# pkusys/Auncel

Hardware: AMD Instinct MI355X
Metric: queries/sec @ recall@10>=0.95, SIFT-10M d=128 IVF4096, 1/2/4/8 GPU (higher is better)
Workload: dtype u8

## Files before the change

### auncel_amd/csrc/ivf_engine.hip

```cpp
#include <hip/hip_runtime.h>

#include <algorithm>
#include <atomic>
#include <cfloat>
#include <cmath>
#include <cstdlib>
#include <chrono>
#include <condition_variable>
#include <deque>
#include <functional>
#include <map>
#include <cstring>
#include <memory>
#include <stdexcept>
#include <string>
#include <mutex>
#include <thread>
#include <unordered_set>
#include <vector>

#include "../../include/auncel_amd.h"
#include "exact_args.h"
#include "ivf_kernels.h"
#include "kmeans_host.h"
// ... 1760 lines not shown
            ra.stage = h->c_stage.as<uint32_t>();
            ra.nscan = h->c_nscan.as<unsigned long long>();
            ra.done = h->c_done.as<uint32_t>();
            ra.D = d_out_dis + c0 * nprobe;
            ra.I = d_out_keys + c0 * nprobe;
            ra.stats = h->w_misc.as<unsigned long long>();
            ra.error = reinterpret_cast<uint32_t*>(h->w_misc.as<unsigned long long>() + STATS_ROWS * 4);
            launch_replay(ra, s);
        } else {
            bool tail_neutral = false;
            if (sort_rows_ranks_a_prefix((uint32_t)nlist, (uint32_t)nprobe, (uint32_t)prefix) && c0 == 0 && m == n && d_out_dis == h->w_cdis.p &&
                d_out_keys == h->w_ckeys.p) {
                amd_ivf::CoarseTail& ct = h->coarse_tail;
                tail_neutral = ct.valid && ct.dis == d_out_dis && ct.keys == d_out_keys && ct.prefix == prefix && ct.nprobe == nprobe && ct.rows >= n &&
                               ct.metric == h->metric && ct.touch_dis + 1 == h->w_cdis.touch && ct.touch_keys + 1 == h->w_ckeys.touch &&
                               !getenv("AUNCEL_AMD_WRITE_TAILS");
                ct = amd_ivf::CoarseTail{true, d_out_dis, d_out_keys, prefix, nprobe, tail_neutral ? ct.rows : n, h->metric, h->w_cdis.touch, h->w_ckeys.touch};
            } else {
                h->coarse_tail.valid = false;
            }
            launch_sort_rows(h->w_dist.as<float>(), (uint32_t)m, (uint32_t)nlist, (uint32_t)nprobe, h->metric,
                             d_out_dis + c0 * nprobe, d_out_keys + c0 * nprobe, s, (uint32_t)prefix, tail_neutral);
            if (heap_ties) {
                if (!h->w_tie_rows.p) {
                    h->w_tie_rows.ensure(8);
                    HIP_CHECK(hipMemsetAsync(h->w_tie_rows.p, 0, 8, s));
                }
                const size_t nout = prefix && prefix < nprobe ? prefix : nprobe;
                const bool ran = launch_heap_tie_order(h->w_dist.as<float>(), (uint32_t)m, (uint32_t)nlist, (uint32_t)nprobe, (uint32_t)nout,
                                                       h->metric, d_out_dis + c0 * nprobe, d_out_keys + c0 * nprobe,
                                                       h->w_tie_rows.as<unsigned long long>(), s);
                if (!ran && (h->ties_override == 1 || ties_opt == 1))
                    throw EngineError("coarse tie order by the reference's heap needs nlist x 12 bytes of LDS (nlist <= ~13 000)");
            }
        }
        h->timer.end(t, s);
        if (!cached || c0 + m < n) {
            HIP_CHECK(stream_sync(s));
            if (c0 == 0 && m == n) {
                h->coarse_sig = csig;
                h->coarse_sig_valid = true;
            }
        }
    }
}

TunerDev make_tuner(amd_ivf* h, size_t query_topk, float multipler, float std_m, const float* d_req, const float* d_gt,
                    unsigned long long* d_np, float* d_tr, int profile) {
    TunerDev t{};
    t.enabled = 1;
    t.profile = profile & 1;
    t.overhead = (profile & 2) ? 1 : 0;
    t.max_topk = (uint32_t)ix(h)->tuner_max_topk;
    t.query_topk = (uint32_t)query_topk;
    t.ntraces = (uint32_t)ix(h)->tuner_ntraces;
    t.multipler = multipler;
    t.std_m = std_m;
    t.interdis = ix(h)->d_interdis.as<float>();
    t.arcos = ix(h)->d_arcos.as<float>();
    t.trace_off = ix(h)->d_trace_off.as<uint32_t>();
    t.trace_x = ix(h)->d_trace_x.as<float>();
    t.trace_y = ix(h)->d_trace_y.as<float>();
    t.trace_std = ix(h)->d_trace_std.as<float>();
    t.require_acc = d_req;
    t.gt_D = d_gt;
    t.my_nprobe = d_np;
    t.t_recalls = d_tr;
    return t;
}

void run_rounds_device(amd_ivf* h, const RoundSpec& base, size_t n, size_t first_round_in, size_t total_nprobe,
                       const unsigned long long* d_np_abs ) {
    amd_ivf* I = ix(h);
    size_t first_round = first_round_in;
    const size_t nlist = h->nlist;
    hipStream_t s = h->stream;
    static const bool sync_env = getenv("AUNCEL_AMD_SYNC_ROUNDS") != nullptr || getenv("AUNCEL_AMD_DEBUG_REPLAY") != nullptr;
    const bool chained = !(base.range || base.d_budget_ms || sync_env);
    const double grow_env = opt(h, OPT_ROUND_GROW, 0.0);
    const bool filter_ok = filter_available(h, I, base.bytes) && !base.range;
    const bool filter_half = filter_ok && ensure_frag16(I);
    if (filter_ok && !filter_half) ensure_frag32(I);
    const float* lanes = base.bytes ? nullptr : ensure_lanes(I);
    struct Fp32Gate {
        amd_ivf* ix;
        bool held;
        Fp32Gate(amd_ivf* index, bool wanted) : ix(index), held(false) {
            if (!wanted || (int)index->opt.get(OPT_FP32_IN_FLIGHT, 4) <= 0) return;
            std::unique_lock<std::mutex> lk(ix->fp32_gate_mu);
            const uint64_t mine = ix->fp32_gate_next++;
            ix->fp32_gate_cv.wait(lk, [&] {
                const int limit = (int)ix->opt.get(OPT_FP32_IN_FLIGHT, 4);
                return mine == ix->fp32_gate_serving && (limit <= 0 || ix->fp32_running < limit);
            });
            ix->fp32_gate_serving++;
            ix->fp32_running++;
            held = true;
            lk.unlock();
            ix->fp32_gate_cv.notify_all();
        }
        ~Fp32Gate() {
            if (!held) return;
            {
                std::lock_guard<std::mutex> lk(ix->fp32_gate_mu);
                ix->fp32_running--;
            }
            ix->fp32_gate_cv.notify_all();
        }
    } fp32_gate(I, !base.bytes && n >= 256);
    if (filter_ok && base.tuner.enabled) first_round = filter_first_probes(I, (size_t)base.k, 64, 0.015);
    const double grow = grow_env > 0 ? grow_env : base.bytes ? 12.0 : filter_ok ? 6.0 : 3.5;
    size_t seg_cap = (size_t)2 << 20;
    if (!base.bytes) {
        const size_t groups = ((size_t)4 << 30) / ((size_t)h->dpad * SCAN_RQ * sizeof(float));
        seg_cap = std::min(seg_cap, std::max<size_t>((size_t)64 << 10, (groups > nlist ? groups - nlist : 0) * SCAN_RQ));
    }
    size_t maxlist = 0;
    for (size_t l = 0; l < nlist; l++) maxlist = std::max<size_t>(maxlist, I->h_list_off[l + 1] - I->h_list_off[l]);
    const size_t item_cap = (seg_cap / 32 + nlist) * ((maxlist + SCAN_WAVE_VECS - 1) / SCAN_WAVE_VECS) + nlist * 4 + 16;
    static const size_t seg_cap_env = getenv("AUNCEL_AMD_SEG_CAP_PAIRS") ? (size_t)atol(getenv("AUNCEL_AMD_SEG_CAP_PAIRS")) : 0;
    const size_t round_pairs = seg_cap_env ? std::min(seg_cap, std::max(seg_cap_env, total_nprobe)) : seg_cap;
    static const size_t budget_env = getenv("AUNCEL_AMD_DIST_BUDGET_MB") ? (size_t)atol(getenv("AUNCEL_AMD_DIST_BUDGET_MB")) << 18 : 0;
    const size_t padded_max = (maxlist + 1023) & ~(size_t)1023;
    const double all_rows = (double)n * (double)std::min<size_t>(total_nprobe, nlist) * (double)padded_max;
    size_t budget = budget_env ? budget_env : std::max<size_t>(h->dist_budget_floats, (size_t)2 << 30);
    const uint64_t bsig = (uint64_t)n * 1000003u ^ (uint64_t)first_round_in * 10007u ^ (uint64_t)total_nprobe * 101u ^ (base.bytes ? 1u : 0u) ^
                          (base.tuner.enabled ? 2u : 0u) ^ (base.train.enabled ? 4u : 0u) ^ ((uint64_t)base.k << 40);
    if (!budget_env && chained && base.tuner.enabled) {
        size_t want;
        size_t known = h->dist_want.get(bsig);
        {
            amd_ivf* owner = ix(h);
            std::lock_guard<std::mutex> lock(owner->want_mu);
            known = std::max(known, owner->shared_want.get(bsig));
        }
        if (known) {
            want = known + known / 4;
        } else {
            const double first = (double)n * (double)std::min<size_t>(std::max<size_t>(first_round_in, 1), std::min<size_t>(total_nprobe, nlist)) * (double)padded_max;
            want = (size_t)std::min<double>(first * (1.0 + 0.25 * grow), (double)budget);
        }
        budget = std::min(budget, std::max<size_t>(want, (size_t)16 << 20));
    }
    if (all_rows < (double)budget) budget = (size_t)all_rows + 64;
    budget = std::max<size_t>(budget, I->h_list_off[nlist] + 1024 * nlist + 1024);
    if (filter_ok && budget > ((size_t)1 << 31)) budget = (size_t)1 << 31;
    if (base.bytes && budget > ((size_t)1 << 31)) throw std::runtime_error("distance rows beyond 2^31 floats (byte-code scan offsets are 32-bit)");
    static const bool no_thr = getenv("AUNCEL_AMD_NO_THRESHOLD") != nullptr;
    h->w_pl_pad.ensure(n * 4);
    h->w_mask.ensure((budget / 64 + 2 + 256) * 8);
    const int row_lists_opt = (int)opt(h, OPT_ROW_LISTS, ROW_LISTS_DEFAULT);
    static const size_t row_lists_min = getenv("AUNCEL_AMD_ROW_LISTS_MIN") ? (size_t)atoi(getenv("AUNCEL_AMD_ROW_LISTS_MIN")) : 256;
    const bool row_lists = row_lists_opt != 0 && n >= row_lists_min;
    if (row_lists) {
        h->w_cl_cnt.ensure(seg_cap * 4);
        h->w_cl_ent.ensure((seg_cap + 64) * CL_CAP * sizeof(uint2));
        h->w_cl_arena.ensure((size_t)CL_ARENA * sizeof(uint2));
        h->w_cl_cursor.ensure(8 * 32 * 4);
    }
    h->w_pl_cnt.ensure(n * 4);
    h->w_pl_need.ensure(n * 8);
    h->w_seg_begin.ensure(n * 4);
    h->w_pl_dist_base.ensure(n * 8);
    h->w_qsel.ensure(n * 4);
    h->w_seg_list.ensure(seg_cap * 4);
    h->w_seg_off.ensure(seg_cap * 8);
    h->w_pair_query.ensure(seg_cap * 4);
    h->w_pair_out.ensure(seg_cap * 8);
    h->w_group_p0.ensure(seg_cap * 4);
    h->w_group_cnt.ensure(seg_cap * 4);
    h->w_items.ensure(item_cap * sizeof(ScanItem));
    h->w_pl_lcount.ensure(nlist * 4);
    h->w_pl_lstart.ensure(nlist * 4);
    h->w_pl_gbase.ensure(nlist * 4);
    h->w_pl_ibase.ensure(4 * nlist * 4);
    h->w_pl_fill.ensure(8 * nlist * 4);
    h->w_seg_slot.ensure(seg_cap * 4);
    constexpr size_t CNT_WORDS = 24 + PLAN_MAX_ROUNDS * 8 + 2;
    constexpr size_t STAT_WORDS = STATS_ROWS * 4 * 2;
    h->w_pl_counters.ensure(CNT_WORDS * 4);
    h->p_counters.ensure((CNT_WORDS + STAT_WORDS) * 4);
    h->w_dist.ensure((budget + 4096) * sizeof(float));
    const size_t log_cap = std::min<size_t>(4096, (std::max<size_t>(256, 32 * (size_t)base.k) + 63) & ~(size_t)63);
    const bool sorted_ok = !base.range && !base.train.enabled && !base.raw_heap_out && base.k <= 128 && I->h_list_off[nlist] < 0xffffffffull &&
                           !h->force_heap_select && opt(h, OPT_SELECT, 1) != 0;
    if (sorted_ok) h->w_log.ensure(n * log_cap * 8);
    const size_t group_cap = seg_cap / SCAN_RQ + nlist;
    if (chained && !base.bytes) h->w_qtile.ensure(group_cap * (size_t)h->dpad * SCAN_RQ * sizeof(float));

    PlanArgs pa{};
    pa.nq = (uint32_t)n;
    pa.nlist = (uint32_t)nlist;
    pa.total_nprobe = (uint32_t)total_nprobe;
    pa.key_stride = base.coarse_stride;
    pa.slot_base = 0;
    pa.first_round = (uint32_t)first_round;
    const size_t inc_env = (size_t)opt(h, OPT_ROUND_INC, 0);
    pa.min_inc = (uint32_t)(inc_env ? inc_env : filter_ok && base.tuner.enabled ? 12 : first_round);
    pa.tune = base.tuner.enabled;
    pa.d = h->d;
    pa.multipler = base.tuner.multipler;
    pa.grow = std::max<double>(base.tuner.multipler, grow);
    pa.id_offset = base.id_offset;
    pa.dist_budget = budget;
    pa.seg_cap = (uint32_t)round_pairs;
    pa.keys = base.d_ckeys;
    pa.list_off = I->d_list_off.as<uint64_t>();
    pa.stage = h->w_stage.as<uint32_t>();
    pa.done = h->w_done.as<uint32_t>();
    pa.my_nprobe = d_np_abs;
    pa.cnt = h->w_pl_cnt.as<uint32_t>();
    pa.need = h->w_pl_need.as<unsigned long long>();
    pa.pad = h->w_pl_pad.as<uint32_t>();
    pa.row_align = sorted_ok ? 1024 : 64;
    h->row_align_now = pa.row_align;
    pa.qblock = scan_qblock(base.bytes);
    pa.mfma_qblock = MFMA_QBLOCK;
    static const int item_order_env = getenv("AUNCEL_AMD_ITEM_ORDER") ? atoi(getenv("AUNCEL_AMD_ITEM_ORDER")) : 0;
    pa.item_order = item_order_env;
    pa.lane_block_off = lanes ? I->d_block_off.as<uint64_t>() : nullptr;
    if (base.bytes) {
        pa.mfma_chunk = mfma_chunk();
        pa.block_off = I->d_block_off.as<uint64_t>();
    }
    constexpr size_t SURV_CAP = (size_t)16 << 20;
    if (filter_ok) {
        h->w_xf.ensure(n * (size_t)filter_steps(h->d) * 8 * sizeof(float));
        h->w_xn.ensure(n * sizeof(float));
        h->w_surv.ensure(SURV_CAP * sizeof(uint4));
        h->w_surv_cnt.ensure(4);
        if (filter_half) {
            h->w_qinfo.ensure(16);
            h->w_fparams.ensure(2 * sizeof(FilterParams));
            HIP_CHECK(hipMemsetAsync(h->w_qinfo.p, 0, 16, s));
            launch_amax(base.d_x, n, h->dpad, h->w_qinfo.as<uint32_t>(), s);
            launch_filter_queries16(base.d_x, n, h->d, h->dpad, h->metric, h->w_qinfo.as<uint32_t>(), I->d_yinfo.as<uint32_t>(),
                                    h->w_xf.as<float>(), h->w_xn.as<float>(), h->w_fparams.as<FilterParams>(), s);
        } else {
            launch_filter_queries(base.d_x, n, h->d, h->dpad, h->metric, h->w_xf.as<float>(), h->w_xn.as<float>(), s);
        }
    }
    pa.seg_begin = h->w_seg_begin.as<uint32_t>();
    pa.dist_base = h->w_pl_dist_base.as<unsigned long long>();
    pa.qsel = h->w_qsel.as<uint32_t>();
    pa.seg_list = h->w_seg_list.as<int32_t>();
    pa.seg_off = h->w_seg_off.as<uint64_t>();
    pa.lcount = h->w_pl_lcount.as<uint32_t>();
    pa.lstart = h->w_pl_lstart.as<uint32_t>();
    pa.gbase = h->w_pl_gbase.as<uint32_t>();
    pa.ibase = h->w_pl_ibase.as<uint32_t>();
    pa.xcount = h->w_pl_fill.as<uint32_t>();
    pa.seg_slot = h->w_seg_slot.as<uint32_t>();
    pa.pair_query = h->w_pair_query.as<uint32_t>();
    pa.pair_out = h->w_pair_out.as<uint64_t>();
    pa.group_p0 = h->w_group_p0.as<uint32_t>();
    pa.group_cnt = h->w_group_cnt.as<uint32_t>();
    pa.items = h->w_items.as<ScanItem>();
    pa.item_cap = (uint32_t)item_cap;
    pa.counters = h->w_pl_counters.as<uint32_t>();
    pa.cl_cursor = row_lists ? h->w_cl_cursor.as<uint32_t>() : nullptr;
    pa.bytes = reinterpret_cast<double*>(h->w_pl_counters.as<uint32_t>() + 16);
    pa.acc64 = reinterpret_cast<unsigned long long*>(h->w_pl_counters.as<uint32_t>() + 18);
    pa.min_bytes = reinterpret_cast<double*>(h->w_pl_counters.as<uint32_t>() + 22);
    pa.min_bytes_thr = reinterpret_cast<double*>(h->w_pl_counters.as<uint32_t>() + 24 + PLAN_MAX_ROUNDS * 8);
    pa.row_bytes = base.bytes ? mfma_ksteps(h->d) * 32 : (uint32_t)h->dpad * 4;
    pa.error = h->w_error.as<uint32_t>();
    uint32_t* const d_unfinished = h->w_pl_counters.as<uint32_t>() + 24;
    pa.round_unfinished = d_unfinished;
    if (base.d_budget_ms) {
        h->w_limit.ensure(n * 4);
        pa.budget_ms = base.d_budget_ms;
        pa.limit = h->w_limit.as<uint32_t>();
    }

    uint32_t* hc = h->p_counters.as<uint32_t>();
    const uint32_t* dcnt = h->w_pl_counters.as<uint32_t>();
    constexpr size_t MAX_HIST = 32;
    const uint64_t sig = (uint64_t)n * 1000003u ^ (uint64_t)first_round * 10007u ^ (uint64_t)total_nprobe * 101u ^ (base.bytes ? 1u : 0u) ^
                         (base.tuner.enabled ? 2u : 0u) ^ (base.train.enabled ? 4u : 0u) ^ ((uint64_t)base.k << 40);
    if (chained) {
        h->w_pl_hist.ensure(MAX_HIST * 64);
        h->p_hist.ensure(MAX_HIST * 64);
        if (h->hint_sig != sig) h->round_hint.clear();
        h->hint_sig = sig;
    }
    auto hint_of = [&](size_t round, int counter) -> uint32_t {
        return chained && (round + 1) * 16 <= h->round_hint.size() ? h->round_hint[round * 16 + counter] : 0u;
    };
    const std::vector<uint32_t> hints_used = chained ? h->round_hint : std::vector<uint32_t>();
    h->hinted_rounds = h->short_rounds = 0;
    h->filter_launches = 0;
    size_t planned_rounds = 0;
    struct Active {
        std::atomic<int>& c;
        int before;
        explicit Active(std::atomic<int>& cc) : c(cc), before(cc.fetch_add(1)) {}
        ~Active() { c.fetch_sub(1); }
    } active(I->active_searches);
    const int scan_pipelined = (int)opt(h, OPT_SCAN_PIPELINED, 7);
    auto plan_round = [&](size_t round_len) {
        pa.round_len = (uint32_t)round_len;
        pa.dense_round = !(base.range || (planned_rounds > 0 && !no_thr));
        if (base.bytes) {
            pa.mfma_chunk = pa.dense_round || base.range ? mfma_chunk() : mfma_chunk_thr();
            pa.mfma_qblock = pa.dense_round ? MFMA_QBLOCK : mfma_thr_qblock(h->d, scan_pipelined, base.range);
        }
        if (filter_ok) {
            const bool mf = !pa.dense_round;
            pa.mfma_chunk = mf ? filter_item_vectors(h->d) : 0;
            pa.mfma_qblock = mf ? filter_item_queries(h->d) : MFMA_QBLOCK;
            pa.block_off = mf ? I->d_block_off.as<uint64_t>() : nullptr;
            pa.qblock = scan_qblock(mf);
            pa.row_bytes = mf && filter_half ? filter_steps16(h->d) * 32u : (uint32_t)h->dpad * 4;
        }
        pa.history = chained && planned_rounds >= 1 && planned_rounds <= MAX_HIST ? h->w_pl_hist.as<uint32_t>() + (planned_rounds - 1) * 16 : nullptr;
        pa.first_plan = planned_rounds == 0;
        pa.run_dis = base.run_ties && planned_rounds == 0 ? base.d_cdis : nullptr;
        size_t t = h->timer.begin(CAT_PLAN, s);
        launch_plan(pa, s);
        h->timer.end(t, s);
        planned_rounds++;
        h->plan_passes++;
    };
    static const bool xcd_off = getenv("AUNCEL_AMD_NO_XCD_CHUNKS") != nullptr;
    static const int nstreams = getenv("AUNCEL_AMD_SCAN_STREAMS") ? atoi(getenv("AUNCEL_AMD_SCAN_STREAMS")) : 1;

    auto keep_args = [&](bool thr_mode, const uint32_t* counts, size_t round) {
        KeepArgs ka{};
        ka.nseg_dev = counts ? nullptr : dcnt + CNT_SEGMENTS;
        ka.nseg = counts ? counts[CNT_SEGMENTS] : 0;
        const uint32_t seen = hint_of(round, CNT_SEGMENTS);
        ka.nseg_hint = (uint32_t)std::min<size_t>(seg_cap, seen ? (size_t)seen + seen / 8 + 4 : n * std::min<size_t>(total_nprobe, 64));
        ka.nlist = (uint32_t)nlist;
        ka.seg_list = h->w_seg_list.as<int32_t>();
        ka.seg_off = h->w_seg_off.as<uint64_t>();
        ka.list_off = I->d_list_off.as<uint64_t>();
        ka.block_off = I->d_block_off.as<uint64_t>();
        ka.keep = base.keep;
        ka.mask = h->w_mask.as<unsigned long long>();
        ka.write = thr_mode ? 0 : 1;
        return ka;
    };
    auto enqueue_scan = [&](bool thr_mode, const uint32_t* counts, size_t round) {
        if (counts && counts[CNT_PAIRS] == 0) return;
        size_t t = h->timer.begin(thr_mode ? CAT_SCAN_THR : CAT_SCAN, s);
        const KeepArgs ka = base.keep ? keep_args(thr_mode, counts, round) : KeepArgs{};
        if (base.bytes) {
            MfmaScanArgs ma{};
            ma.codes_frag = I->d_frag.as<uint8_t>();
            ma.code_cy = I->d_cy.as<int32_t>();
            ma.queries8 = h->w_x8.as<int8_t>();
            ma.query_cx = h->w_xnorm8.as<int32_t>();
            ma.items = h->w_items.as<ScanItem>();
            ma.pair_query = h->w_pair_query.as<uint32_t>();
            ma.pair_out = h->w_pair_out.as<uint64_t>();
            ma.dist = h->w_dist.as<float>();
            ma.d = h->d;
            ma.metric = h->metric;
            ma.xcd_chunks = xcd_off ? 0 : 1;
            ma.nitems = counts ? counts[CNT_QG8] : 0;
            ma.dev_nitems = counts ? nullptr : dcnt + CNT_QG8;
            ma.hint_nitems = hint_of(round, CNT_QG8);
            ma.pipelined = scan_pipelined;
            static const int scan_debug = getenv("AUNCEL_AMD_SCAN_DEBUG") ? atoi(getenv("AUNCEL_AMD_SCAN_DEBUG")) : 0;
            ma.debug = scan_debug;
            if (thr_mode) {
                ma.thr = h->w_thr.as<float>();
                ma.mask = h->w_mask.as<unsigned long long>();
                ma.exact_mask = base.range;
            }
            static const int scan_on_main = getenv("AUNCEL_AMD_SCAN_ON_MAIN") ? atoi(getenv("AUNCEL_AMD_SCAN_ON_MAIN")) : 1;
            if (scan_on_main > 0 || n < 20) {
                launch_scan_mfma(ma, s);
            } else {
                ensure_aux(h, 3, 3);
                HIP_CHECK(hipEventRecord(h->ev_fork, s));
                HIP_CHECK(hipStreamWaitEvent(h->aux[3], h->ev_fork, 0));
                launch_scan_mfma(ma, h->aux[3]);
                HIP_CHECK(hipEventRecord(h->ev_join[3], h->aux[3]));
                HIP_CHECK(hipStreamWaitEvent(s, h->ev_join[3], 0));
            }
        } else if (filter_ok && thr_mode) {
            FilterScanArgs fa{};
            fa.codes_frag = filter_half ? I->d_frag16.as<float>() : I->d_frag32.as<float>();
            fa.half = filter_half ? 1 : 0;
            fa.params = filter_half ? h->w_fparams.as<float>() : nullptr;
            fa.yn = I->d_yn.as<float>();
            fa.xf = h->w_xf.as<float>();
            fa.xn = h->w_xn.as<float>();
            fa.codes = I->d_codes.as<float>();
            fa.queries = base.d_x;
            fa.items = h->w_items.as<ScanItem>();
            fa.pair_query = h->w_pair_query.as<uint32_t>();
            fa.pair_out = h->w_pair_out.as<uint64_t>();
            fa.dist = h->w_dist.as<float>();
            fa.thr = h->w_thr.as<float>();
            fa.mask = h->w_mask.as<unsigned long long>();
            fa.surv = h->w_surv.as<uint4>();
            fa.surv_count = h->w_surv_cnt.as<uint32_t>();
            fa.surv_cap = (uint32_t)SURV_CAP;
            fa.d = h->d;
            fa.dpad = h->dpad;
            fa.metric = h->metric;
            fa.xcd_chunks = xcd_off ? 0 : 1;
            fa.nitems = counts ? counts[CNT_QG8] : 0;
            fa.dev_nitems = counts ? nullptr : dcnt + CNT_QG8;
            fa.hint_nitems = hint_of(round, CNT_QG8);
            HIP_CHECK(hipMemsetAsync(h->w_surv_cnt.p, 0, 4, s));
            ensure_aux(h, 3, 3);
            HIP_CHECK(hipEventRecord(h->ev_fork, s));
            HIP_CHECK(hipStreamWaitEvent(h->aux[3], h->ev_fork, 0));
            launch_scan_filter(fa, h->aux[3], base.keep ? &ka : nullptr);
            h->filter_launches++;
            HIP_CHECK(hipEventRecord(h->ev_join[3], h->aux[3]));
            HIP_CHECK(hipStreamWaitEvent(s, h->ev_join[3], 0));
        } else {
            const size_t ngroups = counts ? counts[CNT_GROUPS] : group_cap;
            if (counts) h->w_qtile.ensure(ngroups * (size_t)h->dpad * SCAN_RQ * sizeof(float));
            launch_pack_queries(base.d_x, h->w_pair_query.as<uint32_t>(), h->w_group_p0.as<uint32_t>(), h->w_group_cnt.as<uint32_t>(), ngroups,
                                h->dpad, h->w_qtile.as<float>(), s, counts ? nullptr : dcnt + CNT_GROUPS, hint_of(round, CNT_GROUPS));
            ScanArgs sa{};
            sa.qtile = h->w_qtile.as<float>();
            sa.codes = I->d_codes.as<float>();
            sa.lanes = lanes;
            sa.queries = base.d_x;
            sa.items = h->w_items.as<ScanItem>();
            sa.pair_query = h->w_pair_query.as<uint32_t>();
            sa.pair_out = h->w_pair_out.as<uint64_t>();
            sa.dist = h->w_dist.as<float>();
            sa.d = h->dpad;
            sa.metric = h->metric;
            sa.fused = base.fused;
            sa.xcd_chunks = xcd_off ? 0 : 1;
            sa.dev_counts = counts ? nullptr : dcnt;
            sa.hint_qg[0] = hint_of(round, CNT_QG1);
            sa.hint_qg[1] = hint_of(round, CNT_QG2);
            sa.hint_qg[2] = hint_of(round, CNT_QG4);
            sa.hint_qg[3] = hint_of(round, CNT_QG8);
            sa.hint_valid = chained && (round + 1) * 16 <= h->round_hint.size();
            if (thr_mode) {
                sa.thr = h->w_thr.as<float>();
                sa.mask = h->w_mask.as<unsigned long long>();
            }
            size_t n_qg[4] = {0, 0, 0, 0};
            if (counts) {
                n_qg[0] = counts[CNT_QG1];
                n_qg[1] = counts[CNT_QG2];
                n_qg[2] = counts[CNT_QG4];
                n_qg[3] = counts[CNT_QG8];
            }
            const bool use_aux[4] = {nstreams >= 2, nstreams >= 3, nstreams >= 3, true};
            ensure_aux(h, nstreams >= 2 ? 0 : 3, 3);
            HIP_CHECK(hipEventRecord(h->ev_fork, s));
            for (int i = 0; i < 4; i++)
                if (use_aux[i]) HIP_CHECK(hipStreamWaitEvent(h->aux[i], h->ev_fork, 0));
            if (nstreams <= 1) launch_scan(sa, n_qg, h->aux[3], h->aux[3], h->aux[3], h->aux[3]);
            else if (nstreams == 2) launch_scan(sa, n_qg, h->aux[3], h->aux[0], h->aux[0], h->aux[3]);
            else launch_scan(sa, n_qg, h->aux[3], h->aux[0], h->aux[1], h->aux[2]);
            for (int i = 0; i < 4; i++)
                if (use_aux[i]) {
                    HIP_CHECK(hipEventRecord(h->ev_join[i], h->aux[i]));
                    HIP_CHECK(hipStreamWaitEvent(s, h->ev_join[i], 0));
                }
        }
        if (base.keep && !(filter_ok && thr_mode && !base.bytes)) launch_keep_rows(ka, s);
        h->timer.end(t, s);
    };

    bool fix_pending = false, sorted_any = false;
    size_t last_fix_round = 0;
    const int fix_opt = (int)opt(h, OPT_TIE_FIX, -1);
    const float seen_rate = I->tie_rate.load();
    const bool ties_common = seen_rate >= 0.f ? seen_rate > 0.02f : (base.bytes || base.fused);
    const bool eager_fix = fix_opt >= 0 ? fix_opt == 1 : (active.before == 0 && ties_common && n >= 512);
    bool fix_due = false;
    size_t fix_due_round = 0;
    auto tie_fix_args = [&](uint32_t round, int final_pass) {
        TieFixArgs ta{};
        ta.metric = h->metric;
        ta.k = base.k;
        ta.nq = (uint32_t)n;
        ta.nlist = (uint32_t)nlist;
        ta.log = h->w_log.as<uint2>();
        ta.log_cap = (uint32_t)log_cap;
        ta.round = round;
        ta.final_pass = final_pass;
        ta.log_cnt = h->w_log_cnt.as<uint32_t>();
        ta.log_snap = h->w_log_snap.as<uint32_t>();
        ta.fin_round = h->w_fin_round.as<uint32_t>();
        ta.fix_val = h->w_fix_val.as<float>();
        ta.fix_ref = h->w_fix_ref.as<int64_t>();
        ta.fix_pos = h->w_fix_pos.as<uint32_t>();
        ta.tie_flag = h->w_tie_flag.as<uint32_t>();
        ta.list_off = I->d_list_off.as<uint64_t>();
        ta.ids = I->d_ids.as<int64_t>();
        ta.store_pairs = base.store_pairs;
        ta.D = h->out_D ? h->out_D : h->w_D.as<float>();
        ta.I = h->out_I ? h->out_I : h->w_I.as<int64_t>();
        return ta;
    };
    auto enqueue_replay = [&](bool thr_mode, uint32_t nact, bool on_device, size_t round, const uint32_t* only = nullptr,
                              const uint32_t* only_count = nullptr) {
        ReplayArgs ra{};
        ra.metric = h->metric;
        ra.k = base.k;
        ra.nlist = (uint32_t)nlist;
        ra.nq = nact;
        ra.nq_dev = only ? only_count : on_device ? dcnt + CNT_ACTIVE : nullptr;
        ra.nq_hint = on_device && round > 0 ? std::max<uint32_t>(1, nact / 3) : nact;
        ra.qsel = only ? only : h->w_qsel.as<uint32_t>();
        ra.total_nprobe = (uint32_t)total_nprobe;
        ra.round_probes = 0;
        ra.id_offset = base.id_offset;
        ra.dist = h->w_dist.as<float>();
        ra.mask = thr_mode || base.keep ? h->w_mask.as<unsigned long long>() : nullptr;
        ra.thr = no_thr ? nullptr : h->w_thr.as<float>();
        ra.seg_off = h->w_seg_off.as<uint64_t>();
        ra.seg_list = h->w_seg_list.as<int32_t>();
        ra.seg_count = h->w_pl_cnt.as<uint32_t>();
        ra.seg_begin = h->w_seg_begin.as<uint32_t>();
        ra.seg_by_slot = 1;
        ra.list_off = I->d_list_off.as<uint64_t>();
        ra.ids = I->d_ids.as<int64_t>();
        ra.store_pairs = base.store_pairs;
        ra.max_codes = base.max_codes;
        ra.heap_val = h->w_heap_val.as<float>();
        ra.heap_ref = h->w_heap_ref.as<int64_t>();
        ra.stage = h->w_stage.as<uint32_t>();
        ra.nscan = h->w_nscan.as<unsigned long long>();
        ra.done = h->w_done.as<uint32_t>();
        ra.pre_val = h->w_pre_val.as<float>();
        ra.stoped = h->w_stoped.as<uint32_t>();
        ra.dtb = h->w_dtb.as<float>();
        ra.coarse_dis = base.d_cdis;
        ra.coarse_keys = base.d_ckeys;
        ra.coarse_stride = base.coarse_stride;
        ra.trace_cap = (uint32_t)I->tuner_trace_cap;
        ra.D = h->out_D ? h->out_D : h->w_D.as<float>();
        ra.I = h->out_I ? h->out_I : h->w_I.as<int64_t>();
        ra.stats = h->w_stats.as<unsigned long long>();
        ra.error = h->w_error.as<uint32_t>();
        ra.tuner = base.tuner;
        ra.train = base.train;
        ra.limit = base.d_budget_ms ? h->w_limit.as<uint32_t>() : nullptr;
        ra.qstat = h->w_qstat.as<uint2>();
        ra.unfinished = round < PLAN_MAX_ROUNDS ? d_unfinished + round * 8 : nullptr;
        if (sorted_ok) {
            ra.log = h->w_log.as<uint2>();
            ra.log_cap = (uint32_t)log_cap;
            ra.log_cnt = h->w_log_cnt.as<uint32_t>();
            ra.amb = h->w_amb.as<uint32_t>();
            ra.tie_flag = h->w_tie_flag.as<uint32_t>();
            ra.round = (uint32_t)round;
            ra.log_snap = h->w_log_snap.as<uint32_t>();
            ra.nq_total = (uint32_t)n;
            ra.fin_round = h->w_fin_round.as<uint32_t>();
        }
        const bool sorted_now = replay_sorted_applies(ra);
        if (sorted_now && eager_fix && round >= 2) HIP_CHECK(hipStreamWaitEvent(s, h->ev_fix[round & 1], 0));
        static const bool dbg_replay_dev = getenv("AUNCEL_AMD_DEBUG_REPLAY") != nullptr;
        if (dbg_replay_dev) {
            h->w_misc.ensure((size_t)nact * 64);
            HIP_CHECK(hipMemsetAsync(h->w_misc.p, 0, (size_t)nact * 64, s));
            ra.dbg = h->w_misc.as<unsigned long long>();
        }
        {
            size_t t = h->timer.begin(thr_mode ? CAT_SELECT_THR : CAT_SELECT, s);
            if (thr_mode && sorted_now && row_lists && (row_lists_opt > 0 || active.before == 0)) {
                CompactArgs ca{};
                ca.nseg_dev = dcnt + CNT_SEGMENTS;
                ca.nseg_hint = (uint32_t)std::min<size_t>(seg_cap, (size_t)ra.nq_hint * std::min<size_t>(total_nprobe, 160));
                ca.nlist = (uint32_t)nlist;
                ca.seg_list = ra.seg_list;
                ca.seg_off = ra.seg_off;
                ca.list_off = ra.list_off;
                ca.dist = ra.dist;
                ca.mask = ra.mask;
                ca.cl_cnt = h->w_cl_cnt.as<uint32_t>();
                ca.cl_ent = h->w_cl_ent.as<uint2>();
                ca.arena = h->w_cl_arena.as<uint2>();
                const char* arena_env = getenv("AUNCEL_AMD_CL_ARENA");
                ca.arena_per_xcd = (arena_env ? std::min<uint32_t>((uint32_t)atoi(arena_env), CL_ARENA) : CL_ARENA) / 8;
                ca.cursor = h->w_cl_cursor.as<uint32_t>();
                launch_compact_rows(ca, s);
                ra.cl_cnt = ca.cl_cnt;
                ra.cl_ent = ca.cl_ent;
                ra.cl_arena = ca.arena;
            }
            launch_replay(ra, s);
            h->timer.end(t, s);
        }
        sorted_any = sorted_any || sorted_now;
        if (sorted_now && eager_fix) {
            fix_due = true;
            fix_due_round = round;
        }
        if (dbg_replay_dev) {
            fprintf(stderr, "[replay] round %zu: %u queries\n", round, nact);
            print_replay_dbg(h, nact, s);
        }
    };
    auto launch_due_fix = [&]() {
        if (!fix_due) return;
        fix_due = false;
        const size_t round = fix_due_round;
        ensure_context_streams(h);
        TieFixArgs ta = tie_fix_args((uint32_t)round, 0);
        HIP_CHECK(hipEventRecord(h->ev_sel, s));
// ... 3213 lines not shown
```

### auncel_amd/csrc/ivf_kernels.h

```cpp
#pragma once
#include <hip/hip_runtime.h>
#include <stddef.h>
#include <stdint.h>
#include <stdio.h>
#include <stdlib.h>
#include <string.h>

#include <stdexcept>
#include <string>

#include "selector_args.h"

namespace amdivf {

inline void check_launch(const char* what) {
    const hipError_t e = hipGetLastError();
    if (e != hipSuccess) throw std::runtime_error(std::string("kernel launch failed: ") + what + ": " + hipGetErrorString(e));
    static const bool sync_each = getenv("AUNCEL_AMD_SYNC_LAUNCH") != nullptr;
    if (sync_each) {
        fprintf(stderr, "[launch] %.100s\n", what);
        const hipError_t s = hipDeviceSynchronize();
        if (s != hipSuccess) throw std::runtime_error(std::string("kernel failed: ") + what + ": " + hipGetErrorString(s));
    }
}
#define LAUNCH(...)                     \
    do {                                \
        (void)hipGetLastError();        \
        hipLaunchKernelGGL(__VA_ARGS__); \
        ::amdivf::check_launch(#__VA_ARGS__); \
    } while (0)

constexpr int METRIC_IP = 0;
constexpr int METRIC_L2 = 1;

constexpr int SCAN_RQ = 8;
constexpr int SCAN_RV = 2;
#ifndef AUNCEL_SCAN_DC
#define AUNCEL_SCAN_DC 16
#endif
constexpr int SCAN_DC = AUNCEL_SCAN_DC;
constexpr int SCAN_WAVE_VECS = 64 * SCAN_RV;

constexpr int SCAN_VB_BITS = 40;
constexpr uint64_t SCAN_VB_MASK = (1ull << SCAN_VB_BITS) - 1;
inline __host__ __device__ uint64_t scan_vec_base(uint64_t first_vector, uint64_t first_block32_of_list, uint32_t pos_in_list) {
    return first_vector | (((first_block32_of_list >> 1) + pos_in_list / 64u) << SCAN_VB_BITS);
}

struct ScanItem {
    uint64_t vec_base;
    uint32_t nvec;
    uint32_t vec_off;
    uint32_t pair_begin;
    uint32_t npair;
    uint32_t qg;
    uint32_t qgroup;
};

struct ScanArgs {
    const float* codes;
    const float* queries;
    const ScanItem* items;
    const uint32_t* pair_query;
    const uint64_t* pair_out;
    float* dist;
    const float* qtile;
    int d;
    int metric;
    int fused;
    const float* thr;
    unsigned long long* mask;
    int xcd_chunks;
    uint32_t nitems;
    const uint32_t* dev_counts;
    uint32_t hint_qg[4];
    int hint_valid;
    const float* lanes;
};

void launch_scan(const ScanArgs& a, const size_t n_qg[4], hipStream_t s, hipStream_t s2 = nullptr, hipStream_t s1 = nullptr,
                 hipStream_t s4 = nullptr);
void launch_lanes_from_f32(const float* codes, const uint64_t* list_off, const uint64_t* block_off, uint32_t nlist, uint64_t nblocks64, int dpad,
                           float* out, hipStream_t s);
constexpr int CNT_ACTIVE = 0, CNT_SEGMENTS = 1, CNT_PAIRS = 2, CNT_GROUPS = 3, CNT_QG1 = 4, CNT_QG2 = 5, CNT_QG4 = 8, CNT_QG8 = 9;
unsigned resident_grid(unsigned workgroups_per_cu);

void launch_pack_queries(const float* queries, const uint32_t* pair_query, const uint32_t* group_p0, const uint32_t* group_cnt,
                         size_t ngroups, int d, float* qtile, hipStream_t s, const uint32_t* dev_ngroups = nullptr, uint32_t hint = 0);

constexpr uint32_t MFMA_BLOCK = 32;
constexpr uint32_t MFMA_QBLOCK = 32;
uint32_t mfma_chunk();
uint32_t mfma_chunk_thr();
inline __host__ __device__ uint32_t mfma_ksteps(int d) { return (uint32_t)(d + 31) / 32; }
inline __host__ __device__ uint64_t mfma_list_blocks(uint64_t size) { return ((size + 63) / 64) * 2; }

struct MfmaScanArgs {
    const uint8_t* codes_frag;
    const int32_t* code_cy;
    const int8_t* queries8;
    const int32_t* query_cx;
    const ScanItem* items;
    const uint32_t* pair_query;
    const uint64_t* pair_out;
    float* dist;
    const float* thr;
    unsigned long long* mask;
    int d;
    int metric;
    int xcd_chunks;
    uint32_t nitems;
    const uint32_t* dev_nitems;
    uint32_t hint_nitems;
    int debug;
    int exact_mask;
    int pipelined;
};
void launch_scan_mfma(const MfmaScanArgs& a, hipStream_t s);
uint32_t mfma_thr_qblock(int d, int pipelined, bool exact_mask);
void launch_frag_from_f32(const float* codes, const uint64_t* list_off, const uint64_t* block_off, uint32_t nlist, uint64_t nblocks, int d,
                          int dpad, int metric, uint8_t* out, int32_t* cy, hipStream_t s);
void launch_sbytes_from_f32(const float* x, size_t n, int d, int dpad, int metric, int8_t* out, int32_t* cx, hipStream_t s);
inline __host__ __device__ uint32_t filter_steps(int d) {
    const uint32_t j = (uint32_t)(d + 7) / 8;
    return j <= 4 ? 4u : j <= 8 ? 8u : j <= 12 ? 12u : j <= 16 ? 16u : (j + 1u) & ~1u;
}
struct FilterScanArgs {
    const float* codes_frag;
    const float* yn;
    const float* xf;
    const float* xn;
    const float* codes;
    const float* queries;
    const ScanItem* items;
    const uint32_t* pair_query;
    const uint64_t* pair_out;
    float* dist;
    const float* thr;
    unsigned long long* mask;
    uint4* surv;
    uint32_t* surv_count;
    uint32_t surv_cap;
    int d, dpad;
    int metric;
    int xcd_chunks;
    uint32_t nitems;
    const uint32_t* dev_nitems;
    uint32_t hint_nitems;
    int half;
    const float* params;
};
struct FilterParams {
    float sx, ps, C, pad;
};
struct KeepArgs;
void launch_scan_filter(const FilterScanArgs& a, hipStream_t s, const KeepArgs* keep = nullptr);
inline __host__ __device__ uint32_t filter_steps16(int d) {
    const uint32_t j = (uint32_t)(d + 15) / 16;
    return j <= 4 ? 4u : j <= 6 ? 6u : j <= 8 ? 8u : (j + 1u) & ~1u;
}
void launch_amax(const float* x, size_t rows, int stride, uint32_t* info, hipStream_t s);
float filter_half_scale(const uint32_t info[4], int d);
void launch_half_params(const uint32_t* qinfo, const uint32_t* yinfo, int d, FilterParams* params, hipStream_t s);
void launch_frag16_from_f32(const float* codes, const uint64_t* list_off, const uint64_t* block_off, uint32_t nlist, uint64_t nblocks, int d,
                            int dpad, int metric, const uint32_t* info, float* out, float* yn, hipStream_t s);
void launch_filter_queries16(const float* x, size_t n, int d, int dpad, int metric, const uint32_t* qinfo, const uint32_t* yinfo, float* xf,
                             float* xn, FilterParams* params, hipStream_t s);
constexpr uint32_t FILTER_WIDE_QUERIES = 128;
constexpr uint32_t FILTER_WIDE_VECTORS = 128;
uint32_t filter_item_queries(int d);
uint32_t filter_item_vectors(int d);
void launch_frag32_from_f32(const float* codes, const uint64_t* list_off, const uint64_t* block_off, uint32_t nlist, uint64_t nblocks, int d,
                            int dpad, int metric, float* out, float* yn, hipStream_t s);
void launch_filter_queries(const float* x, size_t n, int d, int dpad, int metric, float* xf, float* xn, hipStream_t s);

inline __host__ __device__ int scan_qg_class(uint32_t qg) { return qg == 1 ? 0 : qg == 2 ? 1 : qg == 4 ? 2 : 3; }
constexpr uint32_t SCAN_QBLOCK = 8 * SCAN_RQ;
inline __host__ __device__ uint32_t scan_shape_of(uint32_t r) { return r <= SCAN_RQ ? 1u : r <= 2 * SCAN_RQ ? 2u : r <= 4 * SCAN_RQ ? 4u : 8u; }
inline __host__ __device__ uint32_t scan_tile_vecs(uint32_t qg) { return (qg >= 4 || qg == 1 ? 1u : 4u / qg) * SCAN_WAVE_VECS; }

struct TunerDev {
    int enabled;
    int profile;
    int overhead;
    uint32_t max_topk, query_topk, ntraces;
    float multipler, std_m;
    const float* interdis;
    const float* arcos;
    const uint32_t* trace_off;
    const float *trace_x, *trace_y, *trace_std;
    const float* require_acc;
    const float* gt_D;
    unsigned long long* my_nprobe;
    float* t_recalls;
};

struct TrainDev {
    int enabled;
    uint32_t ntraces;
    const float* interdis;
    const float* arcos;
    const float* gt_D;
    float* const* raw;
};

struct ReplayArgs {
    int metric;
    int k;
    uint32_t nlist;
    uint32_t nq;
    const uint32_t* nq_dev;
    uint32_t nq_hint;
    const uint32_t* qsel;
    uint32_t total_nprobe;
    uint32_t round_probes;
    uint64_t id_offset;
    const float* dist;
    const unsigned long long* mask;
    float* thr;
    const uint64_t* seg_off;
    const int32_t* seg_list;
    const uint32_t* seg_count;
    const uint32_t* seg_begin;
    int seg_by_slot;
    const uint64_t* list_off;
    const int64_t* ids;
    int store_pairs;
    int identity_ids;
    unsigned long long max_codes;
    int finalize_all;
    const uint32_t* limit;
    float* heap_val;
    int64_t* heap_ref;
    uint32_t* stage;
    unsigned long long* nscan;
    uint32_t* done;
    float* pre_val;
    uint32_t* stoped;
    float* dtb;
    const float* coarse_dis;
    const int64_t* coarse_keys;
    uint32_t coarse_stride;
    uint32_t trace_cap;
    float* D;
    int64_t* I;
    unsigned long long* stats;
    uint32_t* error;
    int raw_heap_out;
    long long pair_list = -1;
    unsigned long long* dbg;
    TunerDev tuner;
    TrainDev train;
    uint2* log;
    uint32_t log_cap;
    uint32_t* log_cnt;
    uint32_t* amb;
    uint32_t* tie_flag;
    uint32_t round;
    uint32_t* log_snap;
    uint32_t nq_total;
    uint32_t* fin_round;
    uint2* qstat;
    uint32_t* unfinished;
    const uint32_t* cl_cnt;
    const uint2* cl_ent;
    const uint2* cl_arena;
};

bool replay_sorted_applies(const ReplayArgs& a);
void launch_replay(const ReplayArgs& a, hipStream_t s);

constexpr uint32_t CL_CAP = 8;
constexpr uint32_t CL_WALK = 0xffffffffu;
struct CompactArgs {
    const uint32_t* nseg_dev;
    uint32_t nseg;
    uint32_t nseg_hint;
    uint32_t nlist;
    const int32_t* seg_list;
    const uint64_t* seg_off;
    const uint64_t* list_off;
    const float* dist;
    const unsigned long long* mask;
    uint32_t* cl_cnt;
    uint2* cl_ent;
    uint2* arena;
    uint32_t arena_per_xcd;
    uint32_t* cursor;
};
void launch_compact_rows(const CompactArgs& a, hipStream_t s);

struct TieFixArgs {
    int metric;
    int k;
    uint32_t nq, nlist;
    const uint2* log;
    uint32_t log_cap;
    uint32_t round;
    int final_pass;
    const uint32_t* log_cnt;
    const uint32_t* log_snap;
    const uint32_t* fin_round;
    float* fix_val;
    int64_t* fix_ref;
    uint32_t* fix_pos;
    uint32_t* tie_flag;
    const uint64_t* list_off;
    const int64_t* ids;
    int store_pairs, identity_ids;
    float* D;
    int64_t* I;
};
void launch_tie_fix(const TieFixArgs& a, hipStream_t s);

struct RangeArgs {
    uint32_t nq;
    uint32_t nlist;
    const uint32_t* qsel;
    const uint32_t* seg_count;
    const uint32_t* seg_begin;
    const int32_t* seg_list;
    const uint64_t* seg_off;
    const uint64_t* list_off;
    const int64_t* ids;
    const float* dist;
    const unsigned long long* mask;
    uint32_t* counts;
    const unsigned long long* out_off;
    int64_t* out_labels;
    float* out_dist;
    uint32_t* stage;
    uint32_t* done;
    unsigned long long* stats;
    uint32_t* error;
};
void launch_range_count(const RangeArgs& a, hipStream_t s);
void launch_range_fill(const RangeArgs& a, hipStream_t s);

void launch_set_online(int metric, uint32_t nlist, uint32_t nq, const float* coarse_dis, const int64_t* coarse_keys,
                       uint32_t coarse_stride, const float* interdis, const float* arcos, float* dtb, uint32_t* error, hipStream_t s,
                       const uint32_t* qsel = nullptr, const uint32_t* nq_dev = nullptr);
void launch_partition_qsel(const uint32_t* qsel, const uint32_t* nq_dev, uint32_t nq, const int32_t* slot_of, uint32_t* q_free, uint32_t* q_wait,
                           uint32_t* counts, hipStream_t s);

struct PlanArgs {
    uint32_t nq;
    uint32_t nlist;
    uint32_t total_nprobe;
    uint32_t key_stride;
    uint32_t slot_base;
    uint32_t first_round, round_len;
    uint32_t min_inc;
    int tune;
    int d;
    float multipler;
    double grow;
    unsigned long long id_offset;
    unsigned long long dist_budget;
    uint32_t seg_cap;
    const int64_t* keys;
    const uint64_t* list_off;
    const uint32_t* stage;
    const uint32_t* done;
    const unsigned long long* my_nprobe;
    const float* budget_ms;
    float elapsed_ms;
    uint32_t* limit;
    uint32_t* cnt;
    unsigned long long* need;
    uint32_t* pad;
    uint32_t row_align;
    uint32_t qblock;
    uint32_t mfma_chunk;
    uint32_t mfma_qblock;
    int item_order;
    const uint64_t* block_off;
    const uint64_t* lane_block_off;
    uint32_t* seg_begin;
    unsigned long long* dist_base;
    uint32_t* qsel;
    int32_t* seg_list;
    uint64_t* seg_off;
    uint32_t* lcount;
    uint32_t* lstart;
    uint32_t* gbase;
    uint32_t* ibase;
    uint32_t* xcount;
    uint32_t* seg_slot;
    uint32_t* pair_query;
    uint64_t* pair_out;
    uint32_t* group_p0;
    uint32_t* group_cnt;
    ScanItem* items;
    uint32_t item_cap;
    uint32_t* error;
    unsigned long long* acc64;
    uint32_t* history;
    int first_plan;
    uint32_t* round_unfinished;
    uint32_t* cl_cursor;
    uint32_t* counters;
    double* bytes;
    double* min_bytes;
    double* min_bytes_thr;
    uint32_t row_bytes;
    int dense_round;
    const float* run_dis;
};

void launch_xcd_check(uint32_t* counters, uint32_t nkeys, uint32_t* slot, uint32_t* xcc_of, uint32_t n, hipStream_t s);

constexpr uint32_t PLAN_MAX_ROUNDS = 64;
constexpr uint32_t STATS_ROWS = 9;
void launch_plan(const PlanArgs& a, hipStream_t s);

constexpr uint32_t ERR_ARCOS_DOMAIN = 1;
constexpr uint32_t ERR_COSINE_PRECOND = 2;
constexpr uint32_t ERR_INVALID_KEY = 3;
constexpr uint32_t ERR_ITEM_OVERFLOW = 4;
constexpr uint32_t ERR_LOG_OVERFLOW = 5;

bool sort_rows_ranks_a_prefix(uint32_t nlist, uint32_t nprobe, uint32_t prefix);
// ... 238 lines not shown
```

### auncel_amd/csrc/ivf_kernels.hip

```cpp
#include "ivf_dev.h"

#include <float.h>
#include <algorithm>
#include <stdexcept>
#include <stdlib.h>
#include <string>
#include <type_traits>
#include <utility>

namespace amdivf {

#ifndef AUNCEL_SCAN_PF
#define AUNCEL_SCAN_PF 2
#endif
typedef float f2 __attribute__((ext_vector_type(2)));
constexpr int LDS_ROW = SCAN_DC + 4;

template <int QG> struct ScanShape {
    static constexpr int NT = QG == 8 ? 512 : QG == 1 ? 64 : 256;
    static constexpr int vg = QG >= 4 || QG == 1 ? 1 : 4 / QG;
    static constexpr int tile_vecs = vg * SCAN_WAVE_VECS;
    static constexpr int lds_floats = tile_vecs * LDS_ROW;
};

// ... 273 lines not shown
            }
            const f2 ya[SCAN_RV] = {f2{ya4.x, ya4.y}, f2{yb4.x, yb4.y}};
            const f2 yb[SCAN_RV] = {f2{ya4.z, ya4.w}, f2{yb4.z, yb4.w}};
#pragma unroll
            for (int r = 0; r < SCAN_RQ; r++) {
                const f2 qa = f2{qc[r].x, qc[r].y}, qb = f2{qc[r].z, qc[r].w};
#pragma unroll
                for (int v = 0; v < SCAN_RV; v++) {
                    if (METRIC == METRIC_L2) {
                        const f2 ta = ya[v] - qa, tb = yb[v] - qb;
                        if (FUSED) {
                            acc[r][v][0] = __builtin_elementwise_fma(ta, ta, acc[r][v][0]);
                            acc[r][v][1] = __builtin_elementwise_fma(tb, tb, acc[r][v][1]);
                        } else {
                            acc[r][v][0] += ta * ta;
                            acc[r][v][1] += tb * tb;
                        }
                    } else if (FUSED) {
                        acc[r][v][0] = __builtin_elementwise_fma(ya[v], qa, acc[r][v][0]);
                        acc[r][v][1] = __builtin_elementwise_fma(yb[v], qb, acc[r][v][1]);
                    } else {
                        acc[r][v][0] += ya[v] * qa;
                        acc[r][v][1] += yb[v] * qb;
                    }
                }
            }
        }
    }
#undef LANE_LOAD
    scan_tile_store<METRIC>(a, it, acc, true, qgi, vgi, lane, e_row, e_thr);
}

template <int METRIC, int QG, int ARITH>
__global__ __launch_bounds__(ScanShape<QG>::NT) void scan_lanes_kernel(ScanArgs a) {
    uint32_t n = a.nitems;
    const ScanItem* items = a.items;
    if (a.dev_counts) {
        const uint32_t n1 = a.dev_counts[CNT_QG1], n2 = a.dev_counts[CNT_QG2], n4 = a.dev_counts[CNT_QG4], n8 = a.dev_counts[CNT_QG8];
        n = QG == 1 ? n1 : QG == 2 ? n2 : QG == 4 ? n4 : n8;
        items += QG == 1 ? 0 : QG == 2 ? n1 : QG == 4 ? n1 + n2 : n1 + n2 + n4;
    }
    ItemWalk w(n, a.xcd_chunks);
    for (uint32_t i = w.cur; i < w.end; i += w.step) scan_lanes_one<METRIC, QG, ARITH>(a, items[i]);
}

__device__ __forceinline__ void lanes_from_f32_block(const float* codes, const uint64_t* list_off, const uint64_t* block_off, uint32_t nlist,
                                                            int dpad, float* out, uint64_t blk) {
    const int lane = threadIdx.x;
    uint32_t lo = 0, hi = nlist;
    while (hi - lo > 1) {
        const uint32_t mid = (lo + hi) >> 1;
        if ((block_off[mid] >> 1) <= blk) lo = mid;
        else hi = mid;
    }
    const uint64_t pos = (blk - (block_off[lo] >> 1)) * 64 + lane, size = list_off[lo + 1] - list_off[lo];
    const bool ok = pos < size;
    const float4* src = reinterpret_cast<const float4*>(codes + (list_off[lo] + (ok ? pos : 0)) * (uint64_t)dpad);
    const int nsteps = dpad >> 2;
    float4* dst = reinterpret_cast<float4*>(out) + blk * (uint64_t)nsteps * 64 + lane;
    for (int s = 0; s < nsteps; s++) dst[(size_t)s * 64] = ok ? src[s] : make_float4(0.f, 0.f, 0.f, 0.f);
}
__global__ __launch_bounds__(64) void lanes_from_f32_kernel(const float* codes, const uint64_t* list_off, const uint64_t* block_off, uint32_t nlist,
                                                            int dpad, float* out) {
    lanes_from_f32_block(codes, list_off, block_off, nlist, dpad, out, blockIdx.x);
}
__global__ __launch_bounds__(64) void lanes_from_f32_list_kernel(const float* codes, const uint64_t* list_off, const uint64_t* block_off, uint32_t nlist,
                                                            int dpad, float* out, const uint64_t* blocks) {
    lanes_from_f32_block(codes, list_off, block_off, nlist, dpad, out, blocks[blockIdx.x]);
}

void launch_lanes_from_f32(const float* codes, const uint64_t* list_off, const uint64_t* block_off, uint32_t nlist, uint64_t nblocks64, int dpad,
                           float* out, hipStream_t s) {
    if (nblocks64 == 0) return;
    LAUNCH(lanes_from_f32_kernel, dim3((unsigned)nblocks64), dim3(64), 0, s, codes, list_off, block_off, nlist, dpad, out);
}
void launch_lanes_from_f32_list(const float* codes, const uint64_t* list_off, const uint64_t* block_off, uint32_t nlist, const uint64_t* blocks64,
                                uint64_t nlisted, int dpad, float* out, hipStream_t s) {
    if (nlisted == 0) return;
    LAUNCH(lanes_from_f32_list_kernel, dim3((unsigned)nlisted), dim3(64), 0, s, codes, list_off, block_off, nlist, dpad, out, blocks64);
}

__global__ __launch_bounds__(256) void pack_queries_kernel(const float* queries, const uint32_t* pair_query, const uint32_t* group_p0,
                                                           const uint32_t* group_cnt, int d, float* qtile, uint32_t ngroups,
                                                           const uint32_t* dev_ngroups) {
    if (dev_ngroups) ngroups = *dev_ngroups;
    for (uint32_t g = blockIdx.x; g < ngroups; g += gridDim.x) {
        const uint32_t p0 = group_p0[g], cnt = group_cnt[g];
        float4* out = reinterpret_cast<float4*>(qtile + (size_t)g * d * SCAN_RQ);
        const int nstep = d >> 2;
        for (int idx = threadIdx.x; idx < nstep * SCAN_RQ; idx += 256) {
            const int step = idx / SCAN_RQ, r = idx % SCAN_RQ;
            float4 v = make_float4(0.f, 0.f, 0.f, 0.f);
            if ((uint32_t)r < cnt) v = *reinterpret_cast<const float4*>(queries + (size_t)pair_query[p0 + r] * d + step * 4);
            out[idx] = v;
        }
    }
}

void launch_pack_queries(const float* queries, const uint32_t* pair_query, const uint32_t* group_p0, const uint32_t* group_cnt,
                         size_t ngroups, int d, float* qtile, hipStream_t s, const uint32_t* dev_ngroups, uint32_t hint) {
    if (!ngroups && !dev_ngroups) return;
    const unsigned grid = dev_ngroups ? (hint ? hint + hint / 8 + 8 : resident_grid(16)) : (unsigned)ngroups;
    LAUNCH(pack_queries_kernel, dim3(grid), dim3(256), 0, s, queries, pair_query, group_p0, group_cnt, d, qtile, (uint32_t)ngroups, dev_ngroups);
}

unsigned resident_grid(unsigned per_cu) {
    static const unsigned cus = [] {
        int dev = 0, n = 0;
        if (hipGetDevice(&dev) != hipSuccess || hipDeviceGetAttribute(&n, hipDeviceAttributeMultiprocessorCount, dev) != hipSuccess || n <= 0) n = 256;
        return (unsigned)n;
    }();
    return ((cus * per_cu + 7) / 8) * 8;
}

template <class K> static unsigned blocks_per_cu(K kern, int threads, size_t dyn_lds = 0) {
    int nb = 0;
    if (hipOccupancyMaxActiveBlocksPerMultiprocessor(&nb, kern, threads, dyn_lds) != hipSuccess || nb <= 0) nb = 1;
    return (unsigned)nb;
}

template <int QG> static void launch_scan_qg(ScanArgs a, size_t first, size_t n, hipStream_t s) {
    if (n == 0 && !a.dev_counts) return;
    if (!a.dev_counts) a.items += first;
    a.nitems = (uint32_t)n;
    const int threads = ScanShape<QG>::NT;
    const uint32_t hint = a.hint_qg[scan_qg_class(QG)];
    auto go = [&](auto kern) {
        static const unsigned per_cu = blocks_per_cu(kern, threads);
        const unsigned hinted = ((unsigned)((size_t)hint + hint / 8 + 7) / 8) * 8 + 8;
        const dim3 grid((unsigned)(a.dev_counts ? (hint ? hinted : a.hint_valid ? resident_grid(1) : resident_grid(per_cu)) : a.xcd_chunks ? ((n + 7) / 8) * 8 : n)), block(threads);
        LAUNCH(kern, grid, block, 0, s, a);
    };
    if (a.lanes) {
        if (a.metric == METRIC_L2) {
            if (a.fused) go(scan_lanes_kernel<METRIC_L2, QG, 1>);
            else go(scan_lanes_kernel<METRIC_L2, QG, 0>);
        } else {
            if (a.fused) go(scan_lanes_kernel<METRIC_IP, QG, 1>);
            else go(scan_lanes_kernel<METRIC_IP, QG, 0>);
        }
    } else if (a.metric == METRIC_L2) {
        if (a.fused) go(scan_tiles_kernel<METRIC_L2, QG, 1>);
        else go(scan_tiles_kernel<METRIC_L2, QG, 0>);
    } else {
        if (a.fused) go(scan_tiles_kernel<METRIC_IP, QG, 1>);
        else go(scan_tiles_kernel<METRIC_IP, QG, 0>);
    }
}

void launch_scan(const ScanArgs& a, const size_t n_qg[4], hipStream_t s, hipStream_t s2, hipStream_t s1, hipStream_t s4) {
    launch_scan_qg<8>(a, n_qg[0] + n_qg[1] + n_qg[2], n_qg[3], s);
    launch_scan_qg<4>(a, n_qg[0] + n_qg[1], n_qg[2], s4 ? s4 : s);
    launch_scan_qg<2>(a, n_qg[0], n_qg[1], s2 ? s2 : s);
    launch_scan_qg<1>(a, 0, n_qg[0], s1 ? s1 : s);
}


typedef int v4i __attribute__((ext_vector_type(4)));
typedef int v16i __attribute__((ext_vector_type(16)));
#if defined(AUNCEL_MFMA_NT) && AUNCEL_MFMA_NT
#define MFMA_BLOAD(p) __builtin_nontemporal_load(p)
#else
#define MFMA_BLOAD(p) (*(p))
#endif

template <int METRIC, bool MASKED, int NKS>
#ifndef AUNCEL_MFMA_WAVES
#define AUNCEL_MFMA_WAVES 4
#endif
__global__ __launch_bounds__(256) __attribute__((amdgpu_waves_per_eu(AUNCEL_MFMA_WAVES, 8))) void scan_mfma_kernel(MfmaScanArgs a) {
    __shared__ int s_cx[4][32];
    __shared__ int s_u[4][32];
    __shared__ uint32_t s_row[4][32];
    const int lane = threadIdx.x & 63;
    const int wave = __builtin_amdgcn_readfirstlane(threadIdx.x >> 6);
    const int m = lane & 31, h = lane >> 5;
    const int ks = NKS ? NKS : (int)mfma_ksteps(a.d);
    const size_t qstride = (size_t)ks * 32;
    const uint32_t nitems = a.dev_nitems ? *a.dev_nitems : a.nitems;
    ItemWalk w((nitems + 3) >> 2, a.xcd_chunks);
    for (uint32_t wi = w.cur; wi < w.end; wi += w.step) {
    const uint32_t item_no = wi * 4 + wave;
    if (item_no >= nitems) break;
    const ScanItem it = a.items[item_no];

    const bool qok = (uint32_t)m < it.npair;
    uint32_t qrow = 0;
    unsigned long long row = 0;
    int cx = 0, u = 0x7fffffff;
    if (qok) {
        qrow = a.pair_query[it.pair_begin + m];
        row = a.pair_out[it.pair_begin + m] + it.vec_off;
        cx = a.query_cx[qrow];
        if (MASKED) {
            const float thr = a.thr[qrow];
            if (METRIC == METRIC_L2) {
                const float c = ceilf(thr);
                const int T = !(c > 0.f) ? 0 : (c >= 1073741824.f ? 1073741824 : (int)c);
                u = cx - T;
            } else {
                const float f = floorf(thr);
                const int T = !(f < 1073741824.f) ? 0x7fffffff : (f <= -1073741824.f ? -1073741824 : (int)f);
                u = T == 0x7fffffff ? T : T - cx;
            }
        }
    }
    __builtin_amdgcn_fence(__ATOMIC_ACQ_REL, "wavefront");
    __builtin_amdgcn_wave_barrier();
    if (h == 0) {
        s_cx[wave][m] = cx;
        s_u[wave][m] = u;
        s_row[wave][m] = (uint32_t)row;
    }
    const int8_t* qp = a.queries8 + (size_t)qrow * qstride + (size_t)h * (size_t)(16 * ks);
    v4i af[NKS ? NKS : 1];
    if (NKS) {
#pragma unroll
        for (int s = 0; s < NKS; s++) af[s] = qok ? *reinterpret_cast<const v4i*>(qp + 16 * s) : v4i{0, 0, 0, 0};
    }
    __builtin_amdgcn_fence(__ATOMIC_ACQ_REL, "wavefront");
    __builtin_amdgcn_wave_barrier();
    int ur[16], cxr[16];
    uint32_t rowr[16];
#pragma unroll
    for (int g = 0; g < 4; g++) {
        const v4i tu = *reinterpret_cast<const v4i*>(&s_u[wave][8 * g + 4 * h]);
        const v4i tc = *reinterpret_cast<const v4i*>(&s_cx[wave][8 * g + 4 * h]);
        const v4i tr = *reinterpret_cast<const v4i*>(&s_row[wave][8 * g + 4 * h]);
#pragma unroll
        for (int i = 0; i < 4; i++) {
            ur[4 * g + i] = tu[i];
            cxr[4 * g + i] = tc[i];
            rowr[4 * g + i] = (uint32_t)tr[i];
        }
    }

    const size_t block_bytes = (size_t)ks * 1024;
    const uint32_t nblk = ((it.nvec + 63) >> 6) * 2;
    uint32_t* mask32 = reinterpret_cast<uint32_t*>(a.mask);
    v4i b[NKS ? NKS : 1];
    int cyn = 0;
    auto fetch_block = [&](uint32_t i) {
        const uint64_t blk = it.vec_base + i;
        const uint8_t* bp = a.codes_frag + blk * block_bytes + (size_t)lane * 16;
#pragma unroll
        for (int s = 0; s < (NKS ? NKS : 1); s++) b[s] = MFMA_BLOAD(reinterpret_cast<const v4i*>(bp + (size_t)s * 1024));
        cyn = a.code_cy[blk * 32 + m];
    };
    if (NKS) fetch_block(0);
    for (uint32_t i = 0; i < nblk; i++) {
        v16i acc;
#pragma unroll
        for (int r = 0; r < 16; r++) acc[r] = 0;
        int cy;
        if (NKS) {
            __builtin_amdgcn_sched_barrier(0);
#pragma unroll
            for (int s = 0; s < NKS; s++) acc = __builtin_amdgcn_mfma_i32_32x32x32_i8(af[s], b[s], acc, 0, 0, 0);
            cy = cyn;
            __builtin_amdgcn_sched_barrier(0);
            if (i + 1 < nblk) fetch_block(i + 1);
            __builtin_amdgcn_sched_barrier(0);
        } else {
            const uint64_t blk = it.vec_base + i;
            const uint8_t* bp = a.codes_frag + blk * block_bytes + (size_t)lane * 16;
            cy = a.code_cy[blk * 32 + m];
            for (int s = 0; s < ks; s++) {
                const v4i aq = qok ? *reinterpret_cast<const v4i*>(qp + 16 * s) : v4i{0, 0, 0, 0};
                const v4i b0 = MFMA_BLOAD(reinterpret_cast<const v4i*>(bp + (size_t)s * 1024));
                acc = __builtin_amdgcn_mfma_i32_32x32x32_i8(aq, b0, acc, 0, 0, 0);
            }
        }
        const uint32_t lv = i * 32 + m;
        const bool vok = lv < it.nvec;
        const unsigned long long vmask = __ballot(vok);
        int word = 0;
        static_for(std::make_integer_sequence<int, 16>{}, [&](auto R) {
            constexpr int reg = decltype(R)::value;
            constexpr int q0 = (reg & 3) + 8 * (reg >> 2);
            const int t = METRIC == METRIC_L2 ? 2 * acc[reg] - cy : acc[reg] + cy;
            if (MASKED) {
                const bool keep = t > ur[reg];
                const unsigned long long bal = __ballot(keep) & vmask;
                writelane_c<q0>(word, (uint32_t)bal);
                writelane_c<q0 + 4>(word, (uint32_t)(bal >> 32));
                if (bal && keep && vok) {
                    const int cq = s_cx[wave][q0 + 4 * h];
                    uint32_t off = rowr[reg] + lv;
                    asm volatile("" : "+v"(off));
                    a.dist[off] = (float)(METRIC == METRIC_L2 ? cq - t : cq + t);
                }
            } else {
                const int res = METRIC == METRIC_L2 ? cxr[reg] - t : cxr[reg] + t;
                uint32_t off = rowr[reg] + lv;
                asm volatile("" : "+v"(off));
                if (vok && (uint32_t)(q0 + 4 * h) < it.npair) a.dist[off] = (float)res;
            }
        });
        if (MASKED && lane < 32 && qok) mask32[(row + i * 32) >> 5] = (uint32_t)word;
    }
    }
}

#ifdef AUNCEL_AMD_SCAN_PROF
__device__ unsigned long long g_scan_prof[8];
#define SCAN_PROF_NOW() __builtin_amdgcn_s_memtime()
#else
#define SCAN_PROF_NOW() 0ull
#endif
template <int METRIC, int NKS, bool DENSE>
__global__ __launch_bounds__(256) __attribute__((amdgpu_waves_per_eu(4, 8))) void scan_mfma_thr_kernel(MfmaScanArgs a) {
    static_assert(NKS >= 1 && NKS <= 4, "query operand resident in registers");
    __shared__ int s_init[4][32];
    __shared__ int s_cx[4][32];
    __shared__ int s_u[4][32];
    __shared__ uint32_t s_row[4][32];
    constexpr uint32_t MAX_BLK = 16;
    __shared__ uint32_t s_mask[DENSE ? 1 : 4][DENSE ? 1 : MAX_BLK][32];
    const int lane = threadIdx.x & 63;
    const int wave = __builtin_amdgcn_readfirstlane(threadIdx.x >> 6);
    const int m = lane & 31, h = lane >> 5;
    constexpr size_t qstride = (size_t)NKS * 32;
    constexpr size_t block_bytes = (size_t)NKS * 1024;
    [[maybe_unused]] const unsigned long long pt_start = SCAN_PROF_NOW();
    [[maybe_unused]] unsigned long long pt_wait = 0, pt_work = 0, pt_first = 0, pt_pro = 0, pt_mask = 0, pt_items = 0;
    typedef int v8i __attribute__((ext_vector_type(8)));
    typedef const v8i __attribute__((address_space(4)))* item_cp;
    static_assert(sizeof(ScanItem) == 32, "one s_load_dwordx8 per item header");
    const item_cp items_c = (item_cp)(uintptr_t)a.items;
    struct Hdr {
        uint64_t vec_base;
        uint32_t nvec, vec_off, pair_begin, npair;
    };
    auto load_item = [&](uint32_t n) {
        const v8i t = items_c[n];
        Hdr r;
        r.vec_base = (uint64_t)(uint32_t)t[0] | ((uint64_t)(uint32_t)t[1] << 32);
        r.nvec = (uint32_t)t[2];
        r.vec_off = (uint32_t)t[3];
        r.pair_begin = (uint32_t)t[4];
        r.npair = (uint32_t)t[5];
        return r;
    };
    const uint32_t nitems = a.dev_nitems ? *a.dev_nitems : a.nitems;
    ItemWalk w((nitems + 3) >> 2, a.xcd_chunks);
    uint32_t wi = w.cur;
    if (wi >= w.end || wi * 4 + (uint32_t)wave >= nitems) return;
    auto item_of = [&](uint32_t walk) { return walk * 4 + (uint32_t)wave; };
    auto exists = [&](uint32_t walk) { return walk < w.end && item_of(walk) < nitems; };

    v4i b0[NKS], b1[NKS];
    int cy0 = 0, cy1 = 0;
    auto fetch = [&](v4i (&b)[NKS], int& cy, uint64_t blk) {
        const uint8_t* bp = a.codes_frag + blk * block_bytes + (size_t)lane * 16;
#pragma unroll
        for (int s = 0; s < NKS; s++) b[s] = MFMA_BLOAD(reinterpret_cast<const v4i*>(bp + (size_t)s * 1024));
        cy = a.code_cy[blk * 32 + m];
    };

    Hdr cur = load_item(item_of(wi));
    Hdr nxt = load_item(exists(wi + w.step) ? item_of(wi + w.step) : item_of(wi));
    uint32_t pq, po;
    {
        const uint32_t e = cur.pair_begin + ((uint32_t)m < cur.npair ? (uint32_t)m : 0u);
        pq = a.pair_query[e];
        po = (uint32_t)a.pair_out[e];
    }
    fetch(b0, cy0, cur.vec_base);
    fetch(b1, cy1, cur.vec_base + 1);
    uint32_t* mask32 = reinterpret_cast<uint32_t*>(a.mask);

    for (;;) {
        [[maybe_unused]] const unsigned long long pt_item = SCAN_PROF_NOW();
        const uint32_t wn = wi + w.step;
        const bool has_next = exists(wn);
        const Hdr nn = load_item(exists(wn + w.step) ? item_of(wn + w.step) : item_of(wi));
        const bool qok = (uint32_t)m < cur.npair;
        const uint32_t row = po + cur.vec_off;
        const int8_t* qp = a.queries8 + (size_t)pq * qstride + (size_t)h * (size_t)(16 * NKS);
        v4i af[NKS];
#pragma unroll
        for (int s = 0; s < NKS; s++) af[s] = *reinterpret_cast<const v4i*>(qp + 16 * s);
        const int cx = a.query_cx[pq];
        const float thr = DENSE ? 0.f : a.thr[pq];
        const uint32_t en = has_next ? nxt.pair_begin + ((uint32_t)m < nxt.npair ? (uint32_t)m : 0u) : cur.pair_begin;
        const uint32_t pqn = a.pair_query[en];
        const uint32_t pon = (uint32_t)a.pair_out[en];
        if (!qok) {
#pragma unroll
            for (int s = 0; s < NKS; s++) af[s] = v4i{0, 0, 0, 0};
        }
        int u = 0, init = -1073741824;
        if (qok && !DENSE) {
            if (METRIC == METRIC_L2) {
                const float c = ceilf(thr);
                const int T = !(c > 0.f) ? 0 : (c >= 1073741824.f ? 1073741824 : (int)c);
                u = (cx - T) & ~1;
                init = -(u >> 1);
            } else {
                const float f = floorf(thr);
                const int T = !(f < 1073741824.f) ? 0x7fffffff : (f <= -1073741824.f ? -1073741824 : (int)f);
                if (T != 0x7fffffff) {
                    u = T - cx;
                    init = -u;
                }
            }
        }
        asm volatile("" ::"v"(pqn), "v"(pon));
        __builtin_amdgcn_fence(__ATOMIC_ACQ_REL, "wavefront");
        __builtin_amdgcn_wave_barrier();
        if (h == 0) {
            s_init[wave][m] = init;
            s_cx[wave][m] = cx;
            s_u[wave][m] = u;
            s_row[wave][m] = row;
        }
        __builtin_amdgcn_fence(__ATOMIC_ACQ_REL, "wavefront");
        __builtin_amdgcn_wave_barrier();
        v16i cinit;
#pragma unroll
        for (int g = 0; g < 4; g++) {
            const v4i t = DENSE ? v4i{0, 0, 0, 0} : *reinterpret_cast<const v4i*>(&s_init[wave][8 * g + 4 * h]);
#pragma unroll
            for (int i = 0; i < 4; i++) cinit[4 * g + i] = t[i];
        }

        const uint32_t nblk = ((cur.nvec + 63) >> 6) * 2;
#ifdef AUNCEL_AMD_SCAN_PROF
        {
            asm volatile("" ::"v"(cinit), "v"(af[0]), "v"(af[NKS - 1]));
            const unsigned long long t = SCAN_PROF_NOW();
            if (pt_items == 0) pt_first = t - pt_start;
            else pt_pro += t - pt_item;
            pt_items++;
        }
#endif
        auto step = [&](v4i (&b)[NKS], int& cyv, uint32_t i) {
            __builtin_amdgcn_sched_barrier(0);
#ifdef AUNCEL_AMD_SCAN_PROF
            const unsigned long long t_a = SCAN_PROF_NOW();
            asm volatile("" ::"v"(b[0]), "v"(b[NKS - 1]), "v"(cyv));
            const unsigned long long t_b = SCAN_PROF_NOW();
            pt_wait += t_b - t_a;
#endif
            v16i acc = __builtin_amdgcn_mfma_i32_32x32x32_i8(af[0], b[0], cinit, 0, 0, 0);
#pragma unroll
            for (int s = 1; s < NKS; s++) acc = __builtin_amdgcn_mfma_i32_32x32x32_i8(af[s], b[s], acc, 0, 0, 0);
            const uint32_t lv = i * 32 + m;
            const bool vok = lv < cur.nvec;
            int hc = !vok ? 0x7fffffff : METRIC == METRIC_L2 ? cyv >> 1 : -cyv;
            int cy;
            asm volatile("v_mov_b32 %0, %1" : "=v"(cy) : "v"(cyv));
            asm volatile("" : "+v"(hc));
            __builtin_amdgcn_sched_barrier(0);
            const uint32_t in = i + 2;
            const uint64_t nb = in < nblk ? cur.vec_base + in : has_next ? nxt.vec_base + (in - nblk) : cur.vec_base;
            fetch(b, cyv, nb);
            __builtin_amdgcn_sched_barrier(0);
            if (DENSE) {
                static_for(std::make_integer_sequence<int, 4>{}, [&](auto G) {
                    constexpr int g = decltype(G)::value;
                    const v4i c4 = *reinterpret_cast<const v4i*>(&s_cx[wave][8 * g + 4 * h]);
                    const v4i r4 = *reinterpret_cast<const v4i*>(&s_row[wave][8 * g + 4 * h]);
#pragma unroll
                    for (int i = 0; i < 4; i++) {
                        const int t = METRIC == METRIC_L2 ? 2 * acc[4 * g + i] - cy : acc[4 * g + i] + cy;
                        const int res = METRIC == METRIC_L2 ? c4[i] - t : c4[i] + t;
                        uint32_t off = (uint32_t)r4[i] + lv;
                        asm volatile("" : "+v"(off));
                        if (vok && (uint32_t)(8 * g + 4 * h + i) < cur.npair) a.dist[off] = (float)res;
                    }
                });
#ifdef AUNCEL_AMD_SCAN_PROF
                pt_work += SCAN_PROF_NOW() - t_b;
#endif
                return;
            }
            int word = 0;
            static_for(std::make_integer_sequence<int, 2>{}, [&](auto H) {
                constexpr int r0 = decltype(H)::value * 8;
                unsigned long long bal[8];
#pragma unroll
                for (int r = 0; r < 8; r++) bal[r] = __ballot(acc[r0 + r] > hc);
                static_for(std::make_integer_sequence<int, 8>{}, [&](auto R) {
                    constexpr int reg = r0 + decltype(R)::value;
                    constexpr int q0 = (reg & 3) + 8 * (reg >> 2);
                    const unsigned long long b = bal[reg - r0];
                    if (b != 0) {
                        writelane_c<q0>(word, (uint32_t)b);
                        writelane_c<q0 + 4>(word, (uint32_t)(b >> 32));
                        if (acc[reg] > hc && !(a.debug & 2)) {
                            const int cq = s_cx[wave][q0 + 4 * h], uq = s_u[wave][q0 + 4 * h];
                            const uint32_t off = s_row[wave][q0 + 4 * h] + lv;
                            const int t = METRIC == METRIC_L2 ? 2 * (acc[reg] + (uq >> 1)) - cy : acc[reg] + uq + cy;
                            a.dist[off] = (float)(METRIC == METRIC_L2 ? cq - t : cq + t);
                        }
                    }
                });
            });
            if (lane < 32) s_mask[DENSE ? 0 : wave][DENSE ? 0 : i][lane] = (uint32_t)word;
#ifdef AUNCEL_AMD_SCAN_PROF
            asm volatile("" ::"v"(word));
            pt_work += SCAN_PROF_NOW() - t_b;
#endif
        };
        for (uint32_t i = 0; i < nblk; i += 2) {
            step(b0, cy0, i);
            step(b1, cy1, i + 1);
        }
        [[maybe_unused]] const unsigned long long pt_m0 = SCAN_PROF_NOW();
        if (!DENSE) {
            __builtin_amdgcn_fence(__ATOMIC_ACQ_REL, "wavefront");
            __builtin_amdgcn_wave_barrier();
            if (lane < 32 && qok && !(a.debug & 1)) {
                uint32_t* dst = mask32 + (row >> 5);
                for (uint32_t i = 0; i < nblk; i += 4) {
                    if (i + 4 <= nblk) {
                        typedef int v4i8 __attribute__((ext_vector_type(4), aligned(8)));
                        v4i8 t;
#pragma unroll
                        for (int c = 0; c < 4; c++) t[c] = (int)s_mask[DENSE ? 0 : wave][DENSE ? 0 : i + c][lane];
                        *reinterpret_cast<v4i8*>(dst + i) = t;
                    } else {
                        typedef int v2i __attribute__((ext_vector_type(2)));
                        v2i t;
                        t[0] = (int)s_mask[DENSE ? 0 : wave][DENSE ? 0 : i][lane];
                        t[1] = (int)s_mask[DENSE ? 0 : wave][DENSE ? 0 : i + 1][lane];
                        *reinterpret_cast<v2i*>(dst + i) = t;
                    }
                }
            }
        }
#ifdef AUNCEL_AMD_SCAN_PROF
        pt_mask += SCAN_PROF_NOW() - pt_m0;
#endif
        if (!has_next) break;
        cur = nxt;
        nxt = nn;
        pq = pqn;
        po = pon;
        wi = wn;
    }
#ifdef AUNCEL_AMD_SCAN_PROF
    if (lane == 0) {
        atomicAdd(&g_scan_prof[0], 1ull);
        atomicAdd(&g_scan_prof[1], SCAN_PROF_NOW() - pt_start);
        atomicAdd(&g_scan_prof[2], pt_first);
        atomicAdd(&g_scan_prof[3], pt_wait);
        atomicAdd(&g_scan_prof[4], pt_work);
        atomicAdd(&g_scan_prof[5], pt_pro);
        atomicAdd(&g_scan_prof[6], pt_mask);
        atomicAdd(&g_scan_prof[7], pt_items);
    }
#endif
}

template <int METRIC, int NKS>
__global__ __launch_bounds__(256) __attribute__((amdgpu_waves_per_eu(3, 8))) void scan_mfma_pair_kernel(MfmaScanArgs a) {
    static_assert(NKS >= 1 && NKS <= 4, "query operands resident in registers");
    constexpr uint32_t MAX_BLK = 16;
    __shared__ int s_init[4][64];
    __shared__ int s_cx[4][64];
    __shared__ int s_u[4][64];
    __shared__ uint32_t s_row[4][64];
    __shared__ uint32_t s_mask[4][MAX_BLK][64];
    const int lane = threadIdx.x & 63;
    const int wave = __builtin_amdgcn_readfirstlane(threadIdx.x >> 6);
    const int m = lane & 31, h = lane >> 5;
    constexpr size_t qstride = (size_t)NKS * 32;
    constexpr size_t block_bytes = (size_t)NKS * 1024;
    typedef int v8i __attribute__((ext_vector_type(8)));
    typedef const v8i __attribute__((address_space(4)))* item_cp;
    const item_cp items_c = (item_cp)(uintptr_t)a.items;
    struct Hdr {
        uint64_t vec_base;
        uint32_t nvec, vec_off, pair_begin, npair;
    };
    auto load_item = [&](uint32_t n) {
        const v8i t = items_c[n];
        Hdr r;
        r.vec_base = (uint64_t)(uint32_t)t[0] | ((uint64_t)(uint32_t)t[1] << 32);
        r.nvec = (uint32_t)t[2];
        r.vec_off = (uint32_t)t[3];
        r.pair_begin = (uint32_t)t[4];
        r.npair = (uint32_t)t[5];
        return r;
    };
    const uint32_t nitems = a.dev_nitems ? *a.dev_nitems : a.nitems;
    ItemWalk w((nitems + 3) >> 2, a.xcd_chunks);
    uint32_t wi = w.cur;
    if (wi >= w.end || wi * 4 + (uint32_t)wave >= nitems) return;
    auto item_of = [&](uint32_t walk) { return walk * 4 + (uint32_t)wave; };
    auto exists = [&](uint32_t walk) { return walk < w.end && item_of(walk) < nitems; };

    v4i b0[NKS], b1[NKS];
    int cy0 = 0, cy1 = 0;
    auto fetch = [&](v4i (&b)[NKS], int& cy, uint64_t blk) {
        const uint8_t* bp = a.codes_frag + blk * block_bytes + (size_t)lane * 16;
#pragma unroll
        for (int s = 0; s < NKS; s++) b[s] = MFMA_BLOAD(reinterpret_cast<const v4i*>(bp + (size_t)s * 1024));
        cy = a.code_cy[blk * 32 + m];
    };

    Hdr cur = load_item(item_of(wi));
    Hdr nxt = load_item(exists(wi + w.step) ? item_of(wi + w.step) : item_of(wi));
    uint32_t pq, po;
    {
        const uint32_t e = cur.pair_begin + ((uint32_t)lane < cur.npair ? (uint32_t)lane : 0u);
        pq = a.pair_query[e];
        po = (uint32_t)a.pair_out[e];
    }
    fetch(b0, cy0, cur.vec_base);
    fetch(b1, cy1, cur.vec_base + 1);
    uint32_t* mask32 = reinterpret_cast<uint32_t*>(a.mask);

    for (;;) {
        const uint32_t wn = wi + w.step;
        const bool has_next = exists(wn);
        const Hdr nn = load_item(exists(wn + w.step) ? item_of(wn + w.step) : item_of(wi));
        const bool sok = (uint32_t)lane < cur.npair;
        const bool two = cur.npair > 32;
        const uint32_t row = po + cur.vec_off;
        const uint32_t pq0 = (uint32_t)__builtin_amdgcn_ds_bpermute(4 * m, (int)pq);
        const uint32_t pq1 = (uint32_t)__builtin_amdgcn_ds_bpermute(4 * (32 + m), (int)pq);
        const bool qok0 = (uint32_t)m < cur.npair, qok1 = (uint32_t)(32 + m) < cur.npair;
        v4i af0[NKS], af1[NKS];
        {
            const int8_t* q0p = a.queries8 + (size_t)pq0 * qstride + (size_t)h * (size_t)(16 * NKS);
            const int8_t* q1p = a.queries8 + (size_t)pq1 * qstride + (size_t)h * (size_t)(16 * NKS);
#pragma unroll
            for (int s = 0; s < NKS; s++) af0[s] = *reinterpret_cast<const v4i*>(q0p + 16 * s);
#pragma unroll
            for (int s = 0; s < NKS; s++) af1[s] = *reinterpret_cast<const v4i*>(q1p + 16 * s);
        }
        const int cx = a.query_cx[pq];
        const float thr = a.thr[pq];
        const uint32_t en = has_next ? nxt.pair_begin + ((uint32_t)lane < nxt.npair ? (uint32_t)lane : 0u) : cur.pair_begin;
        const uint32_t pqn = a.pair_query[en];
        const uint32_t pon = (uint32_t)a.pair_out[en];
        if (!qok0) {
#pragma unroll
            for (int s = 0; s < NKS; s++) af0[s] = v4i{0, 0, 0, 0};
        }
        if (!qok1) {
#pragma unroll
            for (int s = 0; s < NKS; s++) af1[s] = v4i{0, 0, 0, 0};
        }
        int u = 0, init = -1073741824;
        if (sok) {
            if (METRIC == METRIC_L2) {
                const float c = ceilf(thr);
                const int T = !(c > 0.f) ? 0 : (c >= 1073741824.f ? 1073741824 : (int)c);
                u = (cx - T) & ~1;
                init = -(u >> 1);
            } else {
                const float f = floorf(thr);
                const int T = !(f < 1073741824.f) ? 0x7fffffff : (f <= -1073741824.f ? -1073741824 : (int)f);
                if (T != 0x7fffffff) {
                    u = T - cx;
                    init = -u;
                }
            }
        }
        asm volatile("" ::"v"(pqn), "v"(pon));
        __builtin_amdgcn_fence(__ATOMIC_ACQ_REL, "wavefront");
        __builtin_amdgcn_wave_barrier();
        s_init[wave][lane] = init;
        s_cx[wave][lane] = cx;
        s_u[wave][lane] = u;
        s_row[wave][lane] = row;
        __builtin_amdgcn_fence(__ATOMIC_ACQ_REL, "wavefront");
        __builtin_amdgcn_wave_barrier();

        const uint32_t nblk = ((cur.nvec + 63) >> 6) * 2;
        auto step = [&](v4i (&b)[NKS], int& cyv, uint32_t i) {
            __builtin_amdgcn_sched_barrier(0);
            v16i acc0, acc1;
#pragma unroll
            for (int g = 0; g < 4; g++) {
                const v4i t0 = *reinterpret_cast<const v4i*>(&s_init[wave][8 * g + 4 * h]);
                const v4i t1 = *reinterpret_cast<const v4i*>(&s_init[wave][32 + 8 * g + 4 * h]);
#pragma unroll
                for (int c = 0; c < 4; c++) {
                    acc0[4 * g + c] = t0[c];
                    acc1[4 * g + c] = t1[c];
                }
            }
            if (!(a.debug & 8)) {
#pragma unroll
                for (int s = 0; s < NKS; s++) acc0 = __builtin_amdgcn_mfma_i32_32x32x32_i8(af0[s], b[s], acc0, 0, 0, 0);
                if (two) {
#pragma unroll
                    for (int s = 0; s < NKS; s++) acc1 = __builtin_amdgcn_mfma_i32_32x32x32_i8(af1[s], b[s], acc1, 0, 0, 0);
                }
            } else {
                asm volatile("" ::"v"(b[0]), "v"(b[NKS - 1]));
            }
            const uint32_t lv = i * 32 + m;
            const bool vok = lv < cur.nvec;
            int hc = !vok ? 0x7fffffff : METRIC == METRIC_L2 ? cyv >> 1 : -cyv;
            int cy;
            asm volatile("v_mov_b32 %0, %1" : "=v"(cy) : "v"(cyv));
            asm volatile("" : "+v"(hc));
            __builtin_amdgcn_sched_barrier(0);
            const uint32_t in = i + 2;
            const uint64_t nb = in < nblk ? cur.vec_base + in : has_next ? nxt.vec_base + (in - nblk) : cur.vec_base;
            fetch(b, cyv, nb);
            __builtin_amdgcn_sched_barrier(0);
            int word = 0;
            auto epilogue = [&](const v16i& acc, auto QB) {
                constexpr int qb = decltype(QB)::value;
                static_for(std::make_integer_sequence<int, 2>{}, [&](auto H) {
                    constexpr int r0 = decltype(H)::value * 8;
                    int mx = max(max(acc[r0], acc[r0 + 1]), acc[r0 + 2]);
                    mx = max(max(mx, acc[r0 + 3]), acc[r0 + 4]);
                    mx = max(max(mx, acc[r0 + 5]), acc[r0 + 6]);
                    mx = max(mx, acc[r0 + 7]);
                    if (__ballot(mx > hc) == 0) return;
                    unsigned long long bal[8];
#pragma unroll
                    for (int r = 0; r < 8; r++) bal[r] = __ballot(acc[r0 + r] > hc);
                    static_for(std::make_integer_sequence<int, 8>{}, [&](auto R) {
                        constexpr int reg = r0 + decltype(R)::value;
                        constexpr int q0 = qb + (reg & 3) + 8 * (reg >> 2);
                        const unsigned long long bb = bal[reg - r0];
                        if (bb != 0) {
                            writelane_c<q0>(word, (uint32_t)bb);
                            writelane_c<q0 + 4>(word, (uint32_t)(bb >> 32));
                            if (acc[reg] > hc && !(a.debug & 2)) {
                                const int cq = s_cx[wave][q0 + 4 * h], uq = s_u[wave][q0 + 4 * h];
                                const uint32_t off = s_row[wave][q0 + 4 * h] + lv;
                                const int t = METRIC == METRIC_L2 ? 2 * (acc[reg] + (uq >> 1)) - cy : acc[reg] + uq + cy;
                                a.dist[off] = (float)(METRIC == METRIC_L2 ? cq - t : cq + t);
                            }
                        }
                    });
                });
            };
            if (!(a.debug & 4)) {
                epilogue(acc0, std::integral_constant<int, 0>{});
                if (two) epilogue(acc1, std::integral_constant<int, 32>{});
            }
            s_mask[wave][i][lane] = (uint32_t)word;
        };
        for (uint32_t i = 0; i < nblk; i += 2) {
            step(b0, cy0, i);
            step(b1, cy1, i + 1);
        }
        __builtin_amdgcn_fence(__ATOMIC_ACQ_REL, "wavefront");
        __builtin_amdgcn_wave_barrier();
        if (sok && !(a.debug & 1)) {
            uint32_t* dst = mask32 + (row >> 5);
            for (uint32_t i = 0; i < nblk; i += 4) {
                if (i + 4 <= nblk) {
                    typedef int v4i8 __attribute__((ext_vector_type(4), aligned(8)));
                    v4i8 t;
#pragma unroll
                    for (int c = 0; c < 4; c++) t[c] = (int)s_mask[wave][i + c][lane];
                    *reinterpret_cast<v4i8*>(dst + i) = t;
                } else {
                    typedef int v2i __attribute__((ext_vector_type(2)));
                    v2i t;
                    t[0] = (int)s_mask[wave][i][lane];
                    t[1] = (int)s_mask[wave][i + 1][lane];
                    *reinterpret_cast<v2i*>(dst + i) = t;
                }
            }
        }
        if (!has_next) break;
        cur = nxt;
        nxt = nn;
        pq = pqn;
        po = pon;
        wi = wn;
    }
}

uint32_t mfma_chunk() {
    static const uint32_t v = [] {
        const char* e = getenv("AUNCEL_AMD_MFMA_CHUNK");
        const long x = e ? atol(e) : 0;
        return x >= 64 ? (uint32_t)((x + 63) / 64 * 64) : 256u;
    }();
    return v;
}

uint32_t mfma_chunk_thr() {
    static const uint32_t v = [] {
        const char* e = getenv("AUNCEL_AMD_MFMA_CHUNK_THR");
        const long x = e ? atol(e) : 0;
        return x >= 64 ? (uint32_t)((x + 63) / 64 * 64) : (getenv("AUNCEL_AMD_MFMA_CHUNK") ? mfma_chunk() : 512u);
    }();
    return v;
}

uint32_t mfma_thr_qblock(int d, int pipelined, bool exact_mask) {
    const int ks = (int)mfma_ksteps(d);
    return (pipelined & 4) && !exact_mask && ks >= 1 && ks <= 4 && mfma_chunk() <= 512 && mfma_chunk_thr() <= 512 ? 2 * MFMA_QBLOCK : MFMA_QBLOCK;
}

void launch_scan_mfma(const MfmaScanArgs& a, hipStream_t s) {
    if (a.nitems == 0 && !a.dev_nitems) return;
    const unsigned nwg = (a.nitems + 3) / 4;
    static const unsigned per_cu_env = getenv("AUNCEL_AMD_MFMA_WG_PER_CU") ? (unsigned)atoi(getenv("AUNCEL_AMD_MFMA_WG_PER_CU")) : 0;
    const bool masked = a.thr != nullptr;
    const int ks = (int)mfma_ksteps(a.d);
    static const bool no_hint = getenv("AUNCEL_AMD_RESIDENT_GRIDS") != nullptr;
    auto go = [&](auto kern) {
        static const unsigned per_cu = blocks_per_cu(kern, 256);
        const size_t hwg = ((size_t)a.hint_nitems + a.hint_nitems / 8 + 3) / 4;
        const unsigned hinted = (unsigned)((hwg + 7) / 8) * 8 + 8;
        const dim3 grid(a.dev_nitems ? (a.hint_nitems && !no_hint ? hinted : resident_grid(per_cu_env ? per_cu_env : per_cu))
                                     : a.xcd_chunks ? ((nwg + 7) / 8) * 8 : nwg),
                        block(256);
        LAUNCH(kern, grid, block, 0, s, a);
#ifdef AUNCEL_AMD_SCAN_PROF
        if (getenv("AUNCEL_AMD_SCAN_PROF")) {
            unsigned long long c[8], z[8] = {0, 0, 0, 0, 0, 0, 0, 0};
            (void)hipStreamSynchronize(s);
            (void)hipMemcpyFromSymbol(c, HIP_SYMBOL(g_scan_prof), sizeof c);
            (void)hipMemcpyToSymbol(HIP_SYMBOL(g_scan_prof), z, sizeof z);
            if (c[0])
                fprintf(stderr, "[scan prof] %s grid %u waves %llu items %llu | per wave (cycles of s_memtime): life %.0f first %.0f wait %.0f work %.0f "
                        "item-prologue %.0f mask %.0f\n", masked ? "thr" : "dense", grid.x, c[0], c[7], (double)c[1] / c[0], (double)c[2] / c[0],
                        (double)c[3] / c[0], (double)c[4] / c[0], (double)c[5] / c[0], (double)c[6] / c[0]);
        }
#endif
    };
    auto pick_ks = [&](auto metric, auto msk) {
        constexpr int M = decltype(metric)::value;
        constexpr bool K = decltype(msk)::value;
        switch (ks) {
            case 1: return go(scan_mfma_kernel<M, K, 1>);
            case 2: return go(scan_mfma_kernel<M, K, 2>);
            case 3: return go(scan_mfma_kernel<M, K, 3>);
            case 4: return go(scan_mfma_kernel<M, K, 4>);
            default: return go(scan_mfma_kernel<M, K, 0>);
        }
    };
    if (masked && mfma_thr_qblock(a.d, a.pipelined, a.exact_mask != 0) == 2 * MFMA_QBLOCK) {
        if (a.metric == METRIC_L2) {
            switch (ks) {
                case 1: return go(scan_mfma_pair_kernel<METRIC_L2, 1>);
                case 2: return go(scan_mfma_pair_kernel<METRIC_L2, 2>);
                case 3: return go(scan_mfma_pair_kernel<METRIC_L2, 3>);
                default: return go(scan_mfma_pair_kernel<METRIC_L2, 4>);
            }
        } else {
            switch (ks) {
                case 1: return go(scan_mfma_pair_kernel<METRIC_IP, 1>);
                case 2: return go(scan_mfma_pair_kernel<METRIC_IP, 2>);
                case 3: return go(scan_mfma_pair_kernel<METRIC_IP, 3>);
                default: return go(scan_mfma_pair_kernel<METRIC_IP, 4>);
            }
        }
    }
    if ((a.pipelined & (masked ? 2 : 1)) && !(masked && a.exact_mask) && ks >= 1 && ks <= 4 && mfma_chunk() <= 512 && mfma_chunk_thr() <= 512) {
        auto pick_thr = [&](auto metric, auto dense) {
            constexpr int M = decltype(metric)::value;
            constexpr bool D = decltype(dense)::value;
            switch (ks) {
                case 1: return go(scan_mfma_thr_kernel<M, 1, D>);
                case 2: return go(scan_mfma_thr_kernel<M, 2, D>);
                case 3: return go(scan_mfma_thr_kernel<M, 3, D>);
                default: return go(scan_mfma_thr_kernel<M, 4, D>);
            }
        };
        if (a.metric == METRIC_L2) {
            if (masked) pick_thr(std::integral_constant<int, METRIC_L2>{}, std::false_type{});
            else pick_thr(std::integral_constant<int, METRIC_L2>{}, std::true_type{});
        } else {
            if (masked) pick_thr(std::integral_constant<int, METRIC_IP>{}, std::false_type{});
            else pick_thr(std::integral_constant<int, METRIC_IP>{}, std::true_type{});
        }
        return;
    }
    if (a.metric == METRIC_L2) {
        if (masked) pick_ks(std::integral_constant<int, METRIC_L2>{}, std::true_type{});
        else pick_ks(std::integral_constant<int, METRIC_L2>{}, std::false_type{});
    } else {
        if (masked) pick_ks(std::integral_constant<int, METRIC_IP>{}, std::true_type{});
        else pick_ks(std::integral_constant<int, METRIC_IP>{}, std::false_type{});
    }
}

__device__ __forceinline__ void frag_from_f32_block(const float* codes, const uint64_t* list_off, const uint64_t* block_off, uint32_t nlist,
                                                           int d, int dpad, int metric, uint8_t* out, int32_t* cy, uint64_t blk) {
    const int lane = threadIdx.x, v = lane & 31, h = lane >> 5;
    uint32_t lo = 0, hi = nlist;
    while (hi - lo > 1) {
        const uint32_t mid = (lo + hi) >> 1;
        if (block_off[mid] <= blk) lo = mid;
        else hi = mid;
    }
    const uint64_t pos = (blk - block_off[lo]) * 32 + v, size = list_off[lo + 1] - list_off[lo];
    const bool ok = pos < size;
    const float* src = codes + (list_off[lo] + (ok ? pos : 0)) * (uint64_t)dpad;
    const int ks = (int)mfma_ksteps(d);
    int sq = 0, sum = 0;
    for (int s = 0; s < ks; s++) {
        const int c0 = h * 16 * ks + 16 * s;
        v4i piece;
#pragma unroll
        for (int w = 0; w < 4; w++) {
            uint32_t word = 0;
#pragma unroll
            for (int b = 0; b < 4; b++) {
                const int c = c0 + 4 * w + b;
                int sv = 0;
                if (ok && c < d) {
                    const int uv = (int)src[c];
                    sv = uv - 128;
                    sq += sv * sv;
                    sum += uv;
                }
                word |= (uint32_t)(sv & 0xff) << (8 * b);
            }
            piece[w] = (int)word;
        }
        *reinterpret_cast<v4i*>(out + blk * (uint64_t)ks * 1024 + (uint64_t)s * 1024 + (uint64_t)lane * 16) = piece;
    }
    sq += __shfl_xor(sq, 32);
    sum += __shfl_xor(sum, 32);
    if (h == 0) cy[blk * 32 + v] = !ok ? 0 : metric == METRIC_L2 ? sq : 128 * sum;
}
__global__ __launch_bounds__(64) void frag_from_f32_kernel(const float* codes, const uint64_t* list_off, const uint64_t* block_off, uint32_t nlist,
                                                           int d, int dpad, int metric, uint8_t* out, int32_t* cy) {
    frag_from_f32_block(codes, list_off, block_off, nlist, d, dpad, metric, out, cy, blockIdx.x);
}
__global__ __launch_bounds__(64) void frag_from_f32_list_kernel(const float* codes, const uint64_t* list_off, const uint64_t* block_off, uint32_t nlist,
                                                           int d, int dpad, int metric, uint8_t* out, int32_t* cy, const uint64_t* blocks) {
    frag_from_f32_block(codes, list_off, block_off, nlist, d, dpad, metric, out, cy, blocks[blockIdx.x]);
}

void launch_frag_from_f32(const float* codes, const uint64_t* list_off, const uint64_t* block_off, uint32_t nlist, uint64_t nblocks, int d,
                          int dpad, int metric, uint8_t* out, int32_t* cy, hipStream_t s) {
    if (nblocks == 0) return;
    LAUNCH(frag_from_f32_kernel, dim3((unsigned)nblocks), dim3(64), 0, s, codes, list_off, block_off, nlist, d, dpad, metric, out, cy);
}
void launch_frag_from_f32_list(const float* codes, const uint64_t* list_off, const uint64_t* block_off, uint32_t nlist, const uint64_t* blocks,
                               uint64_t nlisted, int d, int dpad, int metric, uint8_t* out, int32_t* cy, hipStream_t s) {
    if (nlisted == 0) return;
    LAUNCH(frag_from_f32_list_kernel, dim3((unsigned)nlisted), dim3(64), 0, s, codes, list_off, block_off, nlist, d, dpad, metric, out, cy, blocks);
}

__global__ __launch_bounds__(256) void sbytes_from_f32_kernel(const float* x, size_t n, int d, int dpad, int metric, int8_t* out, int32_t* cx) {
    const size_t row = (size_t)blockIdx.x * 4 + (threadIdx.x >> 6);
    const int lane = threadIdx.x & 63;
    if (row >= n) return;
    const int stride = (int)mfma_ksteps(d) * 32;
    int sq = 0, sum = 0;
    for (int c = lane * 4; c < stride; c += 256) {
        uint32_t word = 0;
#pragma unroll
        for (int b = 0; b < 4; b++) {
            int sv = 0;
            if (c + b < d) {
                const int uv = (int)x[row * (size_t)dpad + c + b];
                sv = uv - 128;
                sq += sv * sv;
                sum += uv;
            }
            word |= (uint32_t)(sv & 0xff) << (8 * b);
        }
        *reinterpret_cast<uint32_t*>(out + row * (size_t)stride + c) = word;
    }
    for (int off = 32; off; off >>= 1) {
        sq += __shfl_xor(sq, off);
        sum += __shfl_xor(sum, off);
    }
    if (lane == 0) cx[row] = metric == METRIC_L2 ? sq : 128 * sum - 16384 * d;
}

void launch_sbytes_from_f32(const float* x, size_t n, int d, int dpad, int metric, int8_t* out, int32_t* cx, hipStream_t s) {
    if (n == 0) return;
    LAUNCH(sbytes_from_f32_kernel, dim3((unsigned)((n + 3) / 4)), dim3(256), 0, s, x, n, d, dpad, metric, out, cx);
}

template <bool FILL>
__global__ __launch_bounds__(256) void range_collect_kernel(RangeArgs a) {
    const uint32_t li = blockIdx.x * 4 + (threadIdx.x >> 6);
    const int lane = threadIdx.x & 63;
    if (li >= a.nq) return;
    const uint32_t qi = a.qsel[li];
    const uint32_t cnt = a.seg_count[qi];
    const size_t seg0 = a.seg_begin[qi];
    unsigned long long pos = FILL ? a.out_off[qi] : 0ull;
    unsigned long long nlistv = 0, ndis = 0;
    uint32_t total = 0, err = 0;
    for (uint32_t p = 0; p < cnt; p++) {
        const int key = a.seg_list[seg0 + p];
        if (key < 0) continue;
        if ((uint32_t)key >= a.nlist) {
            err = ERR_INVALID_KEY;
            break;
        }
        const unsigned long long lb = a.list_off[key];
        const uint32_t n = (uint32_t)(a.list_off[key + 1] - lb);
        if (n == 0) continue;
        nlistv++;
        ndis += n;
        const unsigned long long roff = a.seg_off[seg0 + p];
        const unsigned long long* mrow = a.mask + (roff >> 6);
        const uint32_t nchunk = (n + 63) >> 6;
        for (uint32_t w0 = 0; w0 < nchunk; w0 += 64) {
            const unsigned long long word = w0 + lane < nchunk ? mrow[w0 + lane] : 0ull;
            const uint32_t pc = (uint32_t)__builtin_popcountll(word);
            if (!FILL) {
                total += pc;
                continue;
            }
            uint32_t incl = pc;
            for (int off = 1; off < 64; off <<= 1) {
                const uint32_t o = (uint32_t)__shfl_up((int)incl, off);
                if (lane >= off) incl += o;
            }
            unsigned long long o = pos + incl - pc;
            unsigned long long bits = word;
            while (bits) {
                const int b = __builtin_ctzll(bits);
                bits &= bits - 1;
                const uint32_t cand = (w0 + lane) * 64 + b;
                a.out_dist[o] = a.dist[roff + cand];
                a.out_labels[o] = a.ids[lb + cand];
                o++;
            }
            pos += (uint32_t)__shfl((int)incl, 63);
        }
    }
    if (!FILL) {
        for (int off = 32; off; off >>= 1) total += __shfl_xor(total, off);
        if (lane == 0) {
            a.counts[qi] = total;
            a.stage[qi] += cnt;
            a.done[qi] = 1;
            if (nlistv) atomicAdd(&a.stats[0], nlistv);
            if (ndis) atomicAdd(&a.stats[1], ndis);
            if (err) atomicMax(a.error, err);
        }
    }
}

void launch_range_count(const RangeArgs& a, hipStream_t s) {
    if (a.nq) LAUNCH(range_collect_kernel<false>, dim3((a.nq + 3) / 4), dim3(256), 0, s, a);
}
void launch_range_fill(const RangeArgs& a, hipStream_t s) {
    if (a.nq) LAUNCH(range_collect_kernel<true>, dim3((a.nq + 3) / 4), dim3(256), 0, s, a);
}

typedef float f32x16 __attribute__((ext_vector_type(16)));

__global__ __launch_bounds__(256) void row_norms_kernel(const float* x, size_t n, int d, float* out) {
    const size_t i = (size_t)blockIdx.x * 256 + threadIdx.x;
    if (i >= n) return;
    const float4* r = reinterpret_cast<const float4*>(x + i * d);
    float s0 = 0, s1 = 0, s2 = 0, s3 = 0;
    int c = 0;
    for (; c + 3 < d / 4; c += 4) {
        float4 v[4];
#pragma unroll
        for (int u = 0; u < 4; u++) v[u] = r[c + u];
#pragma unroll
        for (int u = 0; u < 4; u++) {
            s0 += v[u].x * v[u].x;
            s1 += v[u].y * v[u].y;
            s2 += v[u].z * v[u].z;
            s3 += v[u].w * v[u].w;
        }
    }
    for (; c < d / 4; c++) {
        const float4 v = r[c];
        s0 += v.x * v.x;
        s1 += v.y * v.y;
        s2 += v.z * v.z;
        s3 += v.w * v.w;
    }
    out[i] = (s0 + s1) + (s2 + s3);
}

constexpr int GEMM_TK = 16, GEMM_LD = 20;

template <int METRIC>
__global__ __launch_bounds__(256) void coarse_gemm_kernel(const float* X, const float* Y, const float* xn, const float* yn, int nq,
                                                          int ny, int d, float* out) {
    __shared__ __align__(16) float As[2][128 * GEMM_LD], Bs[2][128 * GEMM_LD];
    const int tid = threadIdx.x, lane = tid & 63, wave = tid >> 6;
    const int q0 = blockIdx.y * 128, c0 = blockIdx.x * 128;
    const int wq = wave >> 1, wc = wave & 1;
    const int m = lane & 31, h = lane >> 5;
    f32x16 acc[2][2];
#pragma unroll
    for (int i = 0; i < 2; i++)
#pragma unroll
        for (int j = 0; j < 2; j++)
#pragma unroll
            for (int r = 0; r < 16; r++) acc[i][j][r] = 0.f;
    float4 pa[2], pb[2];
    auto fetch = [&](int k0) {
#pragma unroll
        for (int i = 0; i < 2; i++) {
            const int idx = tid + i * 256, row = idx >> 2, c = idx & 3;
            const bool kok = k0 + 4 * c < d;
            pa[i] = q0 + row < nq && kok ? *reinterpret_cast<const float4*>(X + (size_t)(q0 + row) * d + k0 + 4 * c) : make_float4(0.f, 0.f, 0.f, 0.f);
            pb[i] = c0 + row < ny && kok ? *reinterpret_cast<const float4*>(Y + (size_t)(c0 + row) * d + k0 + 4 * c) : make_float4(0.f, 0.f, 0.f, 0.f);
        }
    };
    auto stage = [&](int buf) {
#pragma unroll
        for (int i = 0; i < 2; i++) {
            const int idx = tid + i * 256, row = idx >> 2, c = idx & 3;
            float* ar = &As[buf][row * GEMM_LD + 2 * c];
            float* br = &Bs[buf][row * GEMM_LD + 2 * c];
            *reinterpret_cast<float2*>(ar) = make_float2(pa[i].x, pa[i].z);
            *reinterpret_cast<float2*>(ar + 8) = make_float2(pa[i].y, pa[i].w);
            *reinterpret_cast<float2*>(br) = make_float2(pb[i].x, pb[i].z);
            *reinterpret_cast<float2*>(br + 8) = make_float2(pb[i].y, pb[i].w);
        }
    };
    fetch(0);
    stage(0);
    __syncthreads();
    int buf = 0;
    for (int k0 = 0; k0 < d; k0 += GEMM_TK, buf ^= 1) {
        const bool more = k0 + GEMM_TK < d;
        if (more) fetch(k0 + GEMM_TK);
        const float* a_base = &As[buf][(wq * 64 + m) * GEMM_LD + h * 8];
        const float* b_base = &Bs[buf][(wc * 64 + m) * GEMM_LD + h * 8];
#pragma unroll
        for (int j0 = 0; j0 < 8; j0 += 4) {
            const float4 a0 = *reinterpret_cast<const float4*>(a_base + j0), a1 = *reinterpret_cast<const float4*>(a_base + 32 * GEMM_LD + j0);
            const float4 b0 = *reinterpret_cast<const float4*>(b_base + j0), b1 = *reinterpret_cast<const float4*>(b_base + 32 * GEMM_LD + j0);
            const float av0[4] = {a0.x, a0.y, a0.z, a0.w}, av1[4] = {a1.x, a1.y, a1.z, a1.w};
            const float bv0[4] = {b0.x, b0.y, b0.z, b0.w}, bv1[4] = {b1.x, b1.y, b1.z, b1.w};
#pragma unroll
            for (int s = 0; s < 4; s++) {
                acc[0][0] = __builtin_amdgcn_mfma_f32_32x32x2f32(av0[s], bv0[s], acc[0][0], 0, 0, 0);
                acc[0][1] = __builtin_amdgcn_mfma_f32_32x32x2f32(av0[s], bv1[s], acc[0][1], 0, 0, 0);
                acc[1][0] = __builtin_amdgcn_mfma_f32_32x32x2f32(av1[s], bv0[s], acc[1][0], 0, 0, 0);
                acc[1][1] = __builtin_amdgcn_mfma_f32_32x32x2f32(av1[s], bv1[s], acc[1][1], 0, 0, 0);
            }
        }
        if (more) stage(buf ^ 1);
        __syncthreads();
    }
#pragma unroll
    for (int ti = 0; ti < 2; ti++)
#pragma unroll
        for (int tj = 0; tj < 2; tj++)
#pragma unroll
            for (int reg = 0; reg < 16; reg++) {
                const int row = (reg & 3) + 8 * (reg >> 2) + 4 * h, col = m;
                const int q = q0 + wq * 64 + ti * 32 + row, c = c0 + wc * 64 + tj * 32 + col;
                if (q < nq && c < ny) {
                    const float ip = acc[ti][tj][reg];
                    float dis = ip;
                    if (METRIC == METRIC_L2) {
                        dis = xn[q] + yn[c] - 2 * ip;
                        if (dis < 0) dis = 0;
                    }
                    out[(size_t)q * ny + c] = dis;
                }
            }
}

constexpr int GEMM16_TK = 32, GEMM16_LD = 40;
template <int METRIC>
__global__ __launch_bounds__(256) void coarse_gemm16_kernel(const float* X, const float* Y, const float* xn, const float* yn, int nq, int ny,
                                                            int d, float* out, const FilterParams* prm) {
    typedef _Float16 v8h __attribute__((ext_vector_type(8)));
    typedef _Float16 v4h __attribute__((ext_vector_type(4)));
    __shared__ __align__(16) _Float16 As[2][128 * GEMM16_LD], Bs[2][128 * GEMM16_LD];
    const int tid = threadIdx.x, lane = tid & 63, wave = tid >> 6;
    const int q0 = blockIdx.y * 128, c0 = blockIdx.x * 128;
    const int wq = wave >> 1, wc = wave & 1;
    const int m = lane & 31, h = lane >> 5;
    const float sx = prm->sx, sy = prm->pad, ps = prm->ps;
// ... 1003 lines not shown
```

Before: 2.839 million.

## Share 128-query items across a workgroup with LDS-staged query fragments in MFMA scan

```diff
diff --git a/auncel_amd/csrc/ivf_engine.hip b/auncel_amd/csrc/ivf_engine.hip
--- a/auncel_amd/csrc/ivf_engine.hip
+++ b/auncel_amd/csrc/ivf_engine.hip
@@ -2086,8 +2086,9 @@
         pa.round_len = (uint32_t)round_len;
         pa.dense_round = !(base.range || (planned_rounds > 0 && !no_thr));
         if (base.bytes) {
-            pa.mfma_chunk = pa.dense_round || base.range ? mfma_chunk() : mfma_chunk_thr();
-            pa.mfma_qblock = pa.dense_round ? MFMA_QBLOCK : mfma_thr_qblock(h->d, scan_pipelined, base.range);
+            const MfmaItemShape shape = mfma_item_shape(h->d, scan_pipelined, !pa.dense_round, base.range);
+            pa.mfma_chunk = shape.chunk;
+            pa.mfma_qblock = shape.qblock;
         }
         if (filter_ok) {
             const bool mf = !pa.dense_round;
diff --git a/auncel_amd/csrc/ivf_kernels.h b/auncel_amd/csrc/ivf_kernels.h
--- a/auncel_amd/csrc/ivf_kernels.h
+++ b/auncel_amd/csrc/ivf_kernels.h
@@ -90,6 +90,7 @@
 
 constexpr uint32_t MFMA_BLOCK = 32;
 constexpr uint32_t MFMA_QBLOCK = 32;
+constexpr uint32_t MFMA_ITEM_QUERIES = 128;
 uint32_t mfma_chunk();
 uint32_t mfma_chunk_thr();
 inline __host__ __device__ uint32_t mfma_ksteps(int d) { return (uint32_t)(d + 31) / 32; }
@@ -117,7 +118,11 @@
     int pipelined;
 };
 void launch_scan_mfma(const MfmaScanArgs& a, hipStream_t s);
-uint32_t mfma_thr_qblock(int d, int pipelined, bool exact_mask);
+struct MfmaItemShape {
+    uint32_t chunk, qblock;
+    bool shared;
+};
+MfmaItemShape mfma_item_shape(int d, int pipelined, bool masked, bool exact_mask);
 void launch_frag_from_f32(const float* codes, const uint64_t* list_off, const uint64_t* block_off, uint32_t nlist, uint64_t nblocks, int d,
                           int dpad, int metric, uint8_t* out, int32_t* cy, hipStream_t s);
 void launch_sbytes_from_f32(const float* x, size_t n, int d, int dpad, int metric, int8_t* out, int32_t* cx, hipStream_t s);
diff --git a/auncel_amd/csrc/ivf_kernels.hip b/auncel_amd/csrc/ivf_kernels.hip
--- a/auncel_amd/csrc/ivf_kernels.hip
+++ b/auncel_amd/csrc/ivf_kernels.hip
@@ -599,28 +599,24 @@
     }
 }
 
-#ifdef AUNCEL_AMD_SCAN_PROF
-__device__ unsigned long long g_scan_prof[8];
-#define SCAN_PROF_NOW() __builtin_amdgcn_s_memtime()
-#else
-#define SCAN_PROF_NOW() 0ull
-#endif
 template <int METRIC, int NKS, bool DENSE>
-__global__ __launch_bounds__(256) __attribute__((amdgpu_waves_per_eu(4, 8))) void scan_mfma_thr_kernel(MfmaScanArgs a) {
-    static_assert(NKS >= 1 && NKS <= 4, "query operand resident in registers");
-    __shared__ int s_init[4][32];
-    __shared__ int s_cx[4][32];
-    __shared__ int s_u[4][32];
-    __shared__ uint32_t s_row[4][32];
-    constexpr uint32_t MAX_BLK = 16;
-    __shared__ uint32_t s_mask[DENSE ? 1 : 4][DENSE ? 1 : MAX_BLK][32];
+__global__ __launch_bounds__(256) __attribute__((amdgpu_waves_per_eu(3, 8))) void scan_mfma_shared_kernel(MfmaScanArgs a) {
+    static_assert(NKS >= 1 && NKS <= 4, "fragment-ordered query operands of MFMA_ITEM_QUERIES queries within the LDS budget");
+    constexpr uint32_t Q = MFMA_ITEM_QUERIES, NQB = Q / MFMA_QBLOCK;
+    static_assert(Q == 128, "a thread stages one half row of one query; the mask words of a block fill two registers of 64 lanes");
+    __shared__ v4i s_q[NQB * NKS * 64];
+    __shared__ __attribute__((aligned(16))) int s_init[Q];
+    __shared__ __attribute__((aligned(16))) int s_cx[Q];
+    __shared__ __attribute__((aligned(16))) int s_u[Q];
+    __shared__ __attribute__((aligned(16))) uint32_t s_row[Q];
+    constexpr uint32_t FLUSH_BLK = 4;
+    __shared__ uint32_t s_mask[DENSE ? 1 : 4][DENSE ? 1 : FLUSH_BLK][DENSE ? 1 : Q];
     const int lane = threadIdx.x & 63;
     const int wave = __builtin_amdgcn_readfirstlane(threadIdx.x >> 6);
     const int m = lane & 31, h = lane >> 5;
+    const uint32_t sq = threadIdx.x & (Q - 1), shalf = threadIdx.x >> 7;
     constexpr size_t qstride = (size_t)NKS * 32;
     constexpr size_t block_bytes = (size_t)NKS * 1024;
-    [[maybe_unused]] const unsigned long long pt_start = SCAN_PROF_NOW();
-    [[maybe_unused]] unsigned long long pt_wait = 0, pt_work = 0, pt_first = 0, pt_pro = 0, pt_mask = 0, pt_items = 0;
     typedef int v8i __attribute__((ext_vector_type(8)));
     typedef const v8i __attribute__((address_space(4)))* item_cp;
     static_assert(sizeof(ScanItem) == 32, "one s_load_dwordx8 per item header");
@@ -639,12 +635,24 @@
         r.npair = (uint32_t)t[5];
         return r;
     };
+    struct Part {
+        uint64_t base;
+        uint32_t off;
+        uint32_t nblk;
+    };
+    auto part_of = [&](const Hdr& it) {
+        const uint32_t np = (it.nvec + 63) >> 6, per = (np + 3) >> 2, p0 = (uint32_t)wave * per;
+        Part r;
+        r.nblk = p0 < np ? 2 * (np - p0 < per ? np - p0 : per) : 0u;
+        r.off = p0 < np ? 64 * p0 : 0u;
+        r.base = it.vec_base + (r.off >> 5);
+        return r;
+    };
     const uint32_t nitems = a.dev_nitems ? *a.dev_nitems : a.nitems;
-    ItemWalk w((nitems + 3) >> 2, a.xcd_chunks);
+    ItemWalk w(nitems, a.xcd_chunks);
     uint32_t wi = w.cur;
-    if (wi >= w.end || wi * 4 + (uint32_t)wave >= nitems) return;
-    auto item_of = [&](uint32_t walk) { return walk * 4 + (uint32_t)wave; };
-    auto exists = [&](uint32_t walk) { return walk < w.end && item_of(walk) < nitems; };
+    if (wi >= w.end) return;
+    auto exists = [&](uint32_t walk) { return walk < w.end; };
 
     v4i b0[NKS], b1[NKS];
     int cy0 = 0, cy1 = 0;
@@ -655,40 +663,45 @@
         cy = a.code_cy[blk * 32 + m];
     };
 
-    Hdr cur = load_item(item_of(wi));
-    Hdr nxt = load_item(exists(wi + w.step) ? item_of(wi + w.step) : item_of(wi));
+    Hdr cur = load_item(wi);
+    Hdr nxt = load_item(exists(wi + w.step) ? wi + w.step : wi);
     uint32_t pq, po;
     {
-        const uint32_t e = cur.pair_begin + ((uint32_t)m < cur.npair ? (uint32_t)m : 0u);
+        const uint32_t e = cur.pair_begin + (sq < cur.npair ? sq : 0u);
         pq = a.pair_query[e];
         po = (uint32_t)a.pair_out[e];
     }
-    fetch(b0, cy0, cur.vec_base);
-    fetch(b1, cy1, cur.vec_base + 1);
+    {
+        const Part p = part_of(cur);
+        fetch(b0, cy0, p.base);
+        fetch(b1, cy1, p.base + 1);
+    }
     uint32_t* mask32 = reinterpret_cast<uint32_t*>(a.mask);
 
     for (;;) {
-        [[maybe_unused]] const unsigned long long pt_item = SCAN_PROF_NOW();
         const uint32_t wn = wi + w.step;
         const bool has_next = exists(wn);
-        const Hdr nn = load_item(exists(wn + w.step) ? item_of(wn + w.step) : item_of(wi));
-        const bool qok = (uint32_t)m < cur.npair;
-        const uint32_t row = po + cur.vec_off;
-        const int8_t* qp = a.queries8 + (size_t)pq * qstride + (size_t)h * (size_t)(16 * NKS);
-        v4i af[NKS];
-#pragma unroll
-        for (int s = 0; s < NKS; s++) af[s] = *reinterpret_cast<const v4i*>(qp + 16 * s);
+        const Hdr nn = load_item(exists(wn + w.step) ? wn + w.step : wi);
+        const Part part = part_of(cur), npart = part_of(nxt);
+        const uint32_t nqb = (cur.npair + MFMA_QBLOCK - 1) / MFMA_QBLOCK;
+        const bool sok = sq < cur.npair;
+        v4i qa[NKS];
+        {
+            const int8_t* qp = a.queries8 + (size_t)pq * qstride + (size_t)shalf * (size_t)(16 * NKS);
+#pragma unroll
+            for (int s = 0; s < NKS; s++) qa[s] = *reinterpret_cast<const v4i*>(qp + 16 * s);
+        }
         const int cx = a.query_cx[pq];
         const float thr = DENSE ? 0.f : a.thr[pq];
-        const uint32_t en = has_next ? nxt.pair_begin + ((uint32_t)m < nxt.npair ? (uint32_t)m : 0u) : cur.pair_begin;
+        const uint32_t en = has_next ? nxt.pair_begin + (sq < nxt.npair ? sq : 0u) : cur.pair_begin;
         const uint32_t pqn = a.pair_query[en];
         const uint32_t pon = (uint32_t)a.pair_out[en];
-        if (!qok) {
-#pragma unroll
-            for (int s = 0; s < NKS; s++) af[s] = v4i{0, 0, 0, 0};
+        if (!sok) {
+#pragma unroll
+            for (int s = 0; s < NKS; s++) qa[s] = v4i{0, 0, 0, 0};
         }
         int u = 0, init = -1073741824;
-        if (qok && !DENSE) {
+        if (sok && !DENSE) {
             if (METRIC == METRIC_L2) {
                 const float c = ceilf(thr);
                 const int T = !(c > 0.f) ? 0 : (c >= 1073741824.f ? 1073741824 : (int)c);
@@ -704,46 +717,40 @@
             }
         }
         asm volatile("" ::"v"(pqn), "v"(pon));
-        __builtin_amdgcn_fence(__ATOMIC_ACQ_REL, "wavefront");
-        __builtin_amdgcn_wave_barrier();
-        if (h == 0) {
-            s_init[wave][m] = init;
-            s_cx[wave][m] = cx;
-            s_u[wave][m] = u;
-            s_row[wave][m] = row;
-        }
-        __builtin_amdgcn_fence(__ATOMIC_ACQ_REL, "wavefront");
-        __builtin_amdgcn_wave_barrier();
-        v16i cinit;
-#pragma unroll
-        for (int g = 0; g < 4; g++) {
-            const v4i t = DENSE ? v4i{0, 0, 0, 0} : *reinterpret_cast<const v4i*>(&s_init[wave][8 * g + 4 * h]);
-#pragma unroll
-            for (int i = 0; i < 4; i++) cinit[4 * g + i] = t[i];
-        }
-
-        const uint32_t nblk = ((cur.nvec + 63) >> 6) * 2;
-#ifdef AUNCEL_AMD_SCAN_PROF
-        {
-            asm volatile("" ::"v"(cinit), "v"(af[0]), "v"(af[NKS - 1]));
-            const unsigned long long t = SCAN_PROF_NOW();
-            if (pt_items == 0) pt_first = t - pt_start;
-            else pt_pro += t - pt_item;
-            pt_items++;
-        }
-#endif
+        __builtin_amdgcn_fence(__ATOMIC_RELEASE, "workgroup");
+        __builtin_amdgcn_s_barrier();
+#pragma unroll
+        for (int s = 0; s < NKS; s++) s_q[((sq >> 5) * NKS + s) * 64 + shalf * 32 + (sq & 31)] = qa[s];
+        if (shalf == 0) {
+            s_init[sq] = init;
+            s_cx[sq] = cx;
+            s_u[sq] = u;
+            s_row[sq] = po + cur.vec_off;
+        }
+        __builtin_amdgcn_fence(__ATOMIC_RELEASE, "workgroup");
+        __builtin_amdgcn_s_barrier();
+        __builtin_amdgcn_fence(__ATOMIC_ACQUIRE, "workgroup");
+
+        const uint32_t nblk = part.nblk;
         auto step = [&](v4i (&b)[NKS], int& cyv, uint32_t i) {
             __builtin_amdgcn_sched_barrier(0);
-#ifdef AUNCEL_AMD_SCAN_PROF
-            const unsigned long long t_a = SCAN_PROF_NOW();
-            asm volatile("" ::"v"(b[0]), "v"(b[NKS - 1]), "v"(cyv));
-            const unsigned long long t_b = SCAN_PROF_NOW();
-            pt_wait += t_b - t_a;
-#endif
-            v16i acc = __builtin_amdgcn_mfma_i32_32x32x32_i8(af[0], b[0], cinit, 0, 0, 0);
-#pragma unroll
-            for (int s = 1; s < NKS; s++) acc = __builtin_amdgcn_mfma_i32_32x32x32_i8(af[s], b[s], acc, 0, 0, 0);
-            const uint32_t lv = i * 32 + m;
+            v16i acc[NQB];
+            static_for(std::make_integer_sequence<int, (int)NQB>{}, [&](auto G) {
+                constexpr int g = decltype(G)::value;
+                if (g != 0 && (uint32_t)g >= nqb) return;
+#pragma unroll
+                for (int c = 0; c < 4; c++) {
+                    const v4i t = DENSE ? v4i{0, 0, 0, 0} : *reinterpret_cast<const v4i*>(&s_init[32 * g + 8 * c + 4 * h]);
+#pragma unroll
+                    for (int k = 0; k < 4; k++) acc[g][4 * c + k] = t[k];
+                }
+                if (!(a.debug & 8)) {
+#pragma unroll
+                    for (int s = 0; s < NKS; s++) acc[g] = __builtin_amdgcn_mfma_i32_32x32x32_i8(s_q[(g * NKS + s) * 64 + lane], b[s], acc[g], 0, 0, 0);
+                }
+            });
+            if (a.debug & 8) asm volatile("" ::"v"(b[0]), "v"(b[NKS - 1]));
+            const uint32_t lv = part.off + i * 32 + m;
             const bool vok = lv < cur.nvec;
             int hc = !vok ? 0x7fffffff : METRIC == METRIC_L2 ? cyv >> 1 : -cyv;
             int cy;
@@ -751,320 +758,100 @@
             asm volatile("" : "+v"(hc));
             __builtin_amdgcn_sched_barrier(0);
             const uint32_t in = i + 2;
-            const uint64_t nb = in < nblk ? cur.vec_base + in : has_next ? nxt.vec_base + (in - nblk) : cur.vec_base;
+            const uint64_t nb = in < nblk ? part.base + in : has_next ? npart.base + (in - nblk) : cur.vec_base;
             fetch(b, cyv, nb);
             __builtin_amdgcn_sched_barrier(0);
             if (DENSE) {
-                static_for(std::make_integer_sequence<int, 4>{}, [&](auto G) {
+                static_for(std::make_integer_sequence<int, (int)NQB>{}, [&](auto G) {
                     constexpr int g = decltype(G)::value;
-                    const v4i c4 = *reinterpret_cast<const v4i*>(&s_cx[wave][8 * g + 4 * h]);
-                    const v4i r4 = *reinterpret_cast<const v4i*>(&s_row[wave][8 * g + 4 * h]);
-#pragma unroll
-                    for (int i = 0; i < 4; i++) {
-                        const int t = METRIC == METRIC_L2 ? 2 * acc[4 * g + i] - cy : acc[4 * g + i] + cy;
-                        const int res = METRIC == METRIC_L2 ? c4[i] - t : c4[i] + t;
-                        uint32_t off = (uint32_t)r4[i] + lv;
-                        asm volatile("" : "+v"(off));
-                        if (vok && (uint32_t)(8 * g + 4 * h + i) < cur.npair) a.dist[off] = (float)res;
-                    }
+                    if (g != 0 && (uint32_t)g >= nqb) return;
+                    static_for(std::make_integer_sequence<int, 4>{}, [&](auto C) {
+                        constexpr int c = decltype(C)::value;
+                        const v4i c4 = *reinterpret_cast<const v4i*>(&s_cx[32 * g + 8 * c + 4 * h]);
+                        const v4i r4 = *reinterpret_cast<const v4i*>(&s_row[32 * g + 8 * c + 4 * h]);
+#pragma unroll
+                        for (int k = 0; k < 4; k++) {
+                            const int t = METRIC == METRIC_L2 ? 2 * acc[g][4 * c + k] - cy : acc[g][4 * c + k] + cy;
+                            const int res = METRIC == METRIC_L2 ? c4[k] - t : c4[k] + t;
+                            uint32_t off = (uint32_t)r4[k] + lv;
+                            asm volatile("" : "+v"(off));
+                            if (vok && (uint32_t)(32 * g + 8 * c + 4 * h + k) < cur.npair) a.dist[off] = (float)res;
+                        }
+                    });
                 });
-#ifdef AUNCEL_AMD_SCAN_PROF
-                pt_work += SCAN_PROF_NOW() - t_b;
-#endif
                 return;
             }
-            int word = 0;
-            static_for(std::make_integer_sequence<int, 2>{}, [&](auto H) {
-                constexpr int r0 = decltype(H)::value * 8;
-                unsigned long long bal[8];
-#pragma unroll
-                for (int r = 0; r < 8; r++) bal[r] = __ballot(acc[r0 + r] > hc);
-                static_for(std::make_integer_sequence<int, 8>{}, [&](auto R) {
-                    constexpr int reg = r0 + decltype(R)::value;
-                    constexpr int q0 = (reg & 3) + 8 * (reg >> 2);
-                    const unsigned long long b = bal[reg - r0];
-                    if (b != 0) {
-                        writelane_c<q0>(word, (uint32_t)b);
-                        writelane_c<q0 + 4>(word, (uint32_t)(b >> 32));
-                        if (acc[reg] > hc && !(a.debug & 2)) {
-                            const int cq = s_cx[wave][q0 + 4 * h], uq = s_u[wave][q0 + 4 * h];
-                            const uint32_t off = s_row[wave][q0 + 4 * h] + lv;
-                            const int t = METRIC == METRIC_L2 ? 2 * (acc[reg] + (uq >> 1)) - cy : acc[reg] + uq + cy;
-                            a.dist[off] = (float)(METRIC == METRIC_L2 ? cq - t : cq + t);
-                        }
-                    }
-                });
-            });
-            if (lane < 32) s_mask[DENSE ? 0 : wave][DENSE ? 0 : i][lane] = (uint32_t)word;
-#ifdef AUNCEL_AMD_SCAN_PROF
-            asm volatile("" ::"v"(word));
-            pt_work += SCAN_PROF_NOW() - t_b;
-#endif
-        };
-        for (uint32_t i = 0; i < nblk; i += 2) {
-            step(b0, cy0, i);
-            step(b1, cy1, i + 1);
-        }
-        [[maybe_unused]] const unsigned long long pt_m0 = SCAN_PROF_NOW();
-        if (!DENSE) {
-            __builtin_amdgcn_fence(__ATOMIC_ACQ_REL, "wavefront");
-            __builtin_amdgcn_wave_barrier();
-            if (lane < 32 && qok && !(a.debug & 1)) {
-                uint32_t* dst = mask32 + (row >> 5);
-                for (uint32_t i = 0; i < nblk; i += 4) {
-                    if (i + 4 <= nblk) {
-                        typedef int v4i8 __attribute__((ext_vector_type(4), aligned(8)));
-                        v4i8 t;
-#pragma unroll
-                        for (int c = 0; c < 4; c++) t[c] = (int)s_mask[DENSE ? 0 : wave][DENSE ? 0 : i + c][lane];
-                        *reinterpret_cast<v4i8*>(dst + i) = t;
-                    } else {
-                        typedef int v2i __attribute__((ext_vector_type(2)));
-                        v2i t;
-                        t[0] = (int)s_mask[DENSE ? 0 : wave][DENSE ? 0 : i][lane];
-                        t[1] = (int)s_mask[DENSE ? 0 : wave][DENSE ? 0 : i + 1][lane];
-                        *reinterpret_cast<v2i*>(dst + i) = t;
-                    }
-                }
-            }
-        }
-#ifdef AUNCEL_AMD_SCAN_PROF
-        pt_mask += SCAN_PROF_NOW() - pt_m0;
-#endif
-        if (!has_next) break;
-        cur = nxt;
-        nxt = nn;
-        pq = pqn;
-        po = pon;
-        wi = wn;
-    }
-#ifdef AUNCEL_AMD_SCAN_PROF
-    if (lane == 0) {
-        atomicAdd(&g_scan_prof[0], 1ull);
-        atomicAdd(&g_scan_prof[1], SCAN_PROF_NOW() - pt_start);
-        atomicAdd(&g_scan_prof[2], pt_first);
-        atomicAdd(&g_scan_prof[3], pt_wait);
-        atomicAdd(&g_scan_prof[4], pt_work);
-        atomicAdd(&g_scan_prof[5], pt_pro);
-        atomicAdd(&g_scan_prof[6], pt_mask);
-        atomicAdd(&g_scan_prof[7], pt_items);
-    }
-#endif
-}
-
-template <int METRIC, int NKS>
-__global__ __launch_bounds__(256) __attribute__((amdgpu_waves_per_eu(3, 8))) void scan_mfma_pair_kernel(MfmaScanArgs a) {
-    static_assert(NKS >= 1 && NKS <= 4, "query operands resident in registers");
-    constexpr uint32_t MAX_BLK = 16;
-    __shared__ int s_init[4][64];
-    __shared__ int s_cx[4][64];
-    __shared__ int s_u[4][64];
-    __shared__ uint32_t s_row[4][64];
-    __shared__ uint32_t s_mask[4][MAX_BLK][64];
-    const int lane = threadIdx.x & 63;
-    const int wave = __builtin_amdgcn_readfirstlane(threadIdx.x >> 6);
-    const int m = lane & 31, h = lane >> 5;
-    constexpr size_t qstride = (size_t)NKS * 32;
-    constexpr size_t block_bytes = (size_t)NKS * 1024;
-    typedef int v8i __attribute__((ext_vector_type(8)));
-    typedef const v8i __attribute__((address_space(4)))* item_cp;
-    const item_cp items_c = (item_cp)(uintptr_t)a.items;
-    struct Hdr {
-        uint64_t vec_base;
-        uint32_t nvec, vec_off, pair_begin, npair;
-    };
-    auto load_item = [&](uint32_t n) {
-        const v8i t = items_c[n];
-        Hdr r;
-        r.vec_base = (uint64_t)(uint32_t)t[0] | ((uint64_t)(uint32_t)t[1] << 32);
-        r.nvec = (uint32_t)t[2];
-        r.vec_off = (uint32_t)t[3];
-        r.pair_begin = (uint32_t)t[4];
-        r.npair = (uint32_t)t[5];
-        return r;
-    };
-    const uint32_t nitems = a.dev_nitems ? *a.dev_nitems : a.nitems;
-    ItemWalk w((nitems + 3) >> 2, a.xcd_chunks);
-    uint32_t wi = w.cur;
-    if (wi >= w.end || wi * 4 + (uint32_t)wave >= nitems) return;
-    auto item_of = [&](uint32_t walk) { return walk * 4 + (uint32_t)wave; };
-    auto exists = [&](uint32_t walk) { return walk < w.end && item_of(walk) < nitems; };
-
-    v4i b0[NKS], b1[NKS];
-    int cy0 = 0, cy1 = 0;
-    auto fetch = [&](v4i (&b)[NKS], int& cy, uint64_t blk) {
-        const uint8_t* bp = a.codes_frag + blk * block_bytes + (size_t)lane * 16;
-#pragma unroll
-        for (int s = 0; s < NKS; s++) b[s] = MFMA_BLOAD(reinterpret_cast<const v4i*>(bp + (size_t)s * 1024));
-        cy = a.code_cy[blk * 32 + m];
-    };
-
-    Hdr cur = load_item(item_of(wi));
-    Hdr nxt = load_item(exists(wi + w.step) ? item_of(wi + w.step) : item_of(wi));
-    uint32_t pq, po;
-    {
-        const uint32_t e = cur.pair_begin + ((uint32_t)lane < cur.npair ? (uint32_t)lane : 0u);
-        pq = a.pair_query[e];
-        po = (uint32_t)a.pair_out[e];
-    }
-    fetch(b0, cy0, cur.vec_base);
-    fetch(b1, cy1, cur.vec_base + 1);
-    uint32_t* mask32 = reinterpret_cast<uint32_t*>(a.mask);
-
-    for (;;) {
-        const uint32_t wn = wi + w.step;
-        const bool has_next = exists(wn);
-        const Hdr nn = load_item(exists(wn + w.step) ? item_of(wn + w.step) : item_of(wi));
-        const bool sok = (uint32_t)lane < cur.npair;
-        const bool two = cur.npair > 32;
-        const uint32_t row = po + cur.vec_off;
-        const uint32_t pq0 = (uint32_t)__builtin_amdgcn_ds_bpermute(4 * m, (int)pq);
-        const uint32_t pq1 = (uint32_t)__builtin_amdgcn_ds_bpermute(4 * (32 + m), (int)pq);
-        const bool qok0 = (uint32_t)m < cur.npair, qok1 = (uint32_t)(32 + m) < cur.npair;
-        v4i af0[NKS], af1[NKS];
-        {
-            const int8_t* q0p = a.queries8 + (size_t)pq0 * qstride + (size_t)h * (size_t)(16 * NKS);
-            const int8_t* q1p = a.queries8 + (size_t)pq1 * qstride + (size_t)h * (size_t)(16 * NKS);
-#pragma unroll
-            for (int s = 0; s < NKS; s++) af0[s] = *reinterpret_cast<const v4i*>(q0p + 16 * s);
-#pragma unroll
-            for (int s = 0; s < NKS; s++) af1[s] = *reinterpret_cast<const v4i*>(q1p + 16 * s);
-        }
-        const int cx = a.query_cx[pq];
-        const float thr = a.thr[pq];
-        const uint32_t en = has_next ? nxt.pair_begin + ((uint32_t)lane < nxt.npair ? (uint32_t)lane : 0u) : cur.pair_begin;
-        const uint32_t pqn = a.pair_query[en];
-        const uint32_t pon = (uint32_t)a.pair_out[en];
-        if (!qok0) {
-#pragma unroll
-            for (int s = 0; s < NKS; s++) af0[s] = v4i{0, 0, 0, 0};
-        }
-        if (!qok1) {
-#pragma unroll
-            for (int s = 0; s < NKS; s++) af1[s] = v4i{0, 0, 0, 0};
-        }
-        int u = 0, init = -1073741824;
-        if (sok) {
-            if (METRIC == METRIC_L2) {
-                const float c = ceilf(thr);
-                const int T = !(c > 0.f) ? 0 : (c >= 1073741824.f ? 1073741824 : (int)c);
-                u = (cx - T) & ~1;
-                init = -(u >> 1);
-            } else {
-                const float f = floorf(thr);
-                const int T = !(f < 1073741824.f) ? 0x7fffffff : (f <= -1073741824.f ? -1073741824 : (int)f);
-                if (T != 0x7fffffff) {
-                    u = T - cx;
-                    init = -u;
-                }
-            }
-        }
-        asm volatile("" ::"v"(pqn), "v"(pon));
-        __builtin_amdgcn_fence(__ATOMIC_ACQ_REL, "wavefront");
-        __builtin_amdgcn_wave_barrier();
-        s_init[wave][lane] = init;
-        s_cx[wave][lane] = cx;
-        s_u[wave][lane] = u;
-        s_row[wave][lane] = row;
-        __builtin_amdgcn_fence(__ATOMIC_ACQ_REL, "wavefront");
-        __builtin_amdgcn_wave_barrier();
-
-        const uint32_t nblk = ((cur.nvec + 63) >> 6) * 2;
-        auto step = [&](v4i (&b)[NKS], int& cyv, uint32_t i) {
-            __builtin_amdgcn_sched_barrier(0);
-            v16i acc0, acc1;
-#pragma unroll
-            for (int g = 0; g < 4; g++) {
-                const v4i t0 = *reinterpret_cast<const v4i*>(&s_init[wave][8 * g + 4 * h]);
-                const v4i t1 = *reinterpret_cast<const v4i*>(&s_init[wave][32 + 8 * g + 4 * h]);
-#pragma unroll
-                for (int c = 0; c < 4; c++) {
-                    acc0[4 * g + c] = t0[c];
-                    acc1[4 * g + c] = t1[c];
-                }
-            }
-            if (!(a.debug & 8)) {
-#pragma unroll
-                for (int s = 0; s < NKS; s++) acc0 = __builtin_amdgcn_mfma_i32_32x32x32_i8(af0[s], b[s], acc0, 0, 0, 0);
-                if (two) {
-#pragma unroll
-                    for (int s = 0; s < NKS; s++) acc1 = __builtin_amdgcn_mfma_i32_32x32x32_i8(af1[s], b[s], acc1, 0, 0, 0);
-                }
-            } else {
-                asm volatile("" ::"v"(b[0]), "v"(b[NKS - 1]));
-            }
-            const uint32_t lv = i * 32 + m;
-            const bool vok = lv < cur.nvec;
-            int hc = !vok ? 0x7fffffff : METRIC == METRIC_L2 ? cyv >> 1 : -cyv;
-            int cy;
-            asm volatile("v_mov_b32 %0, %1" : "=v"(cy) : "v"(cyv));
-            asm volatile("" : "+v"(hc));
-            __builtin_amdgcn_sched_barrier(0);
-            const uint32_t in = i + 2;
-            const uint64_t nb = in < nblk ? cur.vec_base + in : has_next ? nxt.vec_base + (in - nblk) : cur.vec_base;
-            fetch(b, cyv, nb);
-            __builtin_amdgcn_sched_barrier(0);
-            int word = 0;
-            auto epilogue = [&](const v16i& acc, auto QB) {
-                constexpr int qb = decltype(QB)::value;
+            int word[2] = {0, 0};
+            static_for(std::make_integer_sequence<int, (int)NQB>{}, [&](auto G) {
+                constexpr int g = decltype(G)::value;
+                if ((g != 0 && (uint32_t)g >= nqb) || (a.debug & 4)) return;
                 static_for(std::make_integer_sequence<int, 2>{}, [&](auto H) {
                     constexpr int r0 = decltype(H)::value * 8;
-                    int mx = max(max(acc[r0], acc[r0 + 1]), acc[r0 + 2]);
-                    mx = max(max(mx, acc[r0 + 3]), acc[r0 + 4]);
-                    mx = max(max(mx, acc[r0 + 5]), acc[r0 + 6]);
-                    mx = max(mx, acc[r0 + 7]);
+                    int mx = max(max(acc[g][r0], acc[g][r0 + 1]), acc[g][r0 + 2]);
+                    mx = max(max(mx, acc[g][r0 + 3]), acc[g][r0 + 4]);
+                    mx = max(max(mx, acc[g][r0 + 5]), acc[g][r0 + 6]);
+                    mx = max(mx, acc[g][r0 + 7]);
                     if (__ballot(mx > hc) == 0) return;
                     unsigned long long bal[8];
 #pragma unroll
-                    for (int r = 0; r < 8; r++) bal[r] = __ballot(acc[r0 + r] > hc);
+                    for (int r = 0; r < 8; r++) bal[r] = __ballot(acc[g][r0 + r] > hc);
                     static_for(std::make_integer_sequence<int, 8>{}, [&](auto R) {
                         constexpr int reg = r0 + decltype(R)::value;
-                        constexpr int q0 = qb + (reg & 3) + 8 * (reg >> 2);
+                        constexpr int q0 = 32 * g + (reg & 3) + 8 * (reg >> 2);
                         const unsigned long long bb = bal[reg - r0];
                         if (bb != 0) {
-                            writelane_c<q0>(word, (uint32_t)bb);
-                            writelane_c<q0 + 4>(word, (uint32_t)(bb >> 32));
-                            if (acc[reg] > hc && !(a.debug & 2)) {
-                                const int cq = s_cx[wave][q0 + 4 * h], uq = s_u[wave][q0 + 4 * h];
-                                const uint32_t off = s_row[wave][q0 + 4 * h] + lv;
-                                const int t = METRIC == METRIC_L2 ? 2 * (acc[reg] + (uq >> 1)) - cy : acc[reg] + uq + cy;
+                            writelane_c<(q0 & 63)>(word[q0 >> 6], (uint32_t)bb);
+                            writelane_c<((q0 + 4) & 63)>(word[q0 >> 6], (uint32_t)(bb >> 32));
+                            if (acc[g][reg] > hc && !(a.debug & 2)) {
+                                const int cq = s_cx[q0 + 4 * h], uq = s_u[q0 + 4 * h];
+                                const uint32_t off = s_row[q0 + 4 * h] + lv;
+                                const int t = METRIC == METRIC_L2 ? 2 * (acc[g][reg] + (uq >> 1)) - cy : acc[g][reg] + uq + cy;
                                 a.dist[off] = (float)(METRIC == METRIC_L2 ? cq - t : cq + t);
                             }
                         }
                     });
                 });
-            };
-            if (!(a.debug & 4)) {
-                epilogue(acc0, std::integral_constant<int, 0>{});
-                if (two) epilogue(acc1, std::integral_constant<int, 32>{});
-            }
-            s_mask[wave][i][lane] = (uint32_t)word;
+            });
+            s_mask[DENSE ? 0 : wave][DENSE ? 0 : i % FLUSH_BLK][DENSE ? 0 : lane] = (uint32_t)word[0];
+            if (nqb > 2) s_mask[DENSE ? 0 : wave][DENSE ? 0 : i % FLUSH_BLK][DENSE ? 0 : 64 + lane] = (uint32_t)word[1];
+        };
+        auto flush = [&](uint32_t i0, uint32_t n) {
+            __builtin_amdgcn_fence(__ATOMIC_ACQ_REL, "wavefront");
+            __builtin_amdgcn_wave_barrier();
+            if (!(a.debug & 1)) {
+                for (uint32_t q = (uint32_t)lane; q < cur.npair; q += 64) {
+                    uint32_t* dst = mask32 + ((s_row[q] + part.off + 32 * i0) >> 5);
+                    if (n == FLUSH_BLK) {
+                        typedef int v4i8 __attribute__((ext_vector_type(4), aligned(8)));
+                        v4i8 t;
+#pragma unroll
+                        for (int c = 0; c < 4; c++) t[c] = (int)s_mask[DENSE ? 0 : wave][DENSE ? 0 : c][DENSE ? 0 : q];
+                        *reinterpret_cast<v4i8*>(dst) = t;
+                    } else {
+                        typedef int v2i __attribute__((ext_vector_type(2)));
+                        v2i t;
+                        t[0] = (int)s_mask[DENSE ? 0 : wave][0][DENSE ? 0 : q];
+                        t[1] = (int)s_mask[DENSE ? 0 : wave][DENSE ? 0 : 1][DENSE ? 0 : q];
+                        *reinterpret_cast<v2i*>(dst) = t;
+                    }
+                }
+            }
+            __builtin_amdgcn_fence(__ATOMIC_ACQ_REL, "wavefront");
+            __builtin_amdgcn_wave_barrier();
         };
         for (uint32_t i = 0; i < nblk; i += 2) {
             step(b0, cy0, i);
             step(b1, cy1, i + 1);
-        }
-        __builtin_amdgcn_fence(__ATOMIC_ACQ_REL, "wavefront");
-        __builtin_amdgcn_wave_barrier();
-        if (sok && !(a.debug & 1)) {
-            uint32_t* dst = mask32 + (row >> 5);
-            for (uint32_t i = 0; i < nblk; i += 4) {
-                if (i + 4 <= nblk) {
-                    typedef int v4i8 __attribute__((ext_vector_type(4), aligned(8)));
-                    v4i8 t;
-#pragma unroll
-                    for (int c = 0; c < 4; c++) t[c] = (int)s_mask[wave][i + c][lane];
-                    *reinterpret_cast<v4i8*>(dst + i) = t;
-                } else {
-                    typedef int v2i __attribute__((ext_vector_type(2)));
-                    v2i t;
-                    t[0] = (int)s_mask[wave][i][lane];
-                    t[1] = (int)s_mask[wave][i + 1][lane];
-                    *reinterpret_cast<v2i*>(dst + i) = t;
-                }
+            if (!DENSE) {
+                if (i & 2) flush(i - 2, FLUSH_BLK);
+                else if (i + 2 >= nblk) flush(i, 2);
             }
         }
         if (!has_next) break;
+        if (nblk == 0) {
+            fetch(b0, cy0, npart.base);
+            fetch(b1, cy1, npart.base + 1);
+        }
         cur = nxt;
         nxt = nn;
         pq = pqn;
@@ -1091,84 +878,57 @@
     return v;
 }
 
-uint32_t mfma_thr_qblock(int d, int pipelined, bool exact_mask) {
+MfmaItemShape mfma_item_shape(int d, int pipelined, bool masked, bool exact_mask) {
     const int ks = (int)mfma_ksteps(d);
-    return (pipelined & 4) && !exact_mask && ks >= 1 && ks <= 4 && mfma_chunk() <= 512 && mfma_chunk_thr() <= 512 ? 2 * MFMA_QBLOCK : MFMA_QBLOCK;
+    const uint32_t chunk = masked && !exact_mask ? mfma_chunk_thr() : mfma_chunk();
+    const bool shared = (pipelined & (masked ? 6 : 1)) && !(masked && exact_mask) && ks >= 1 && ks <= 4 && mfma_chunk() <= 512 && mfma_chunk_thr() <= 512;
+    return shared ? MfmaItemShape{4 * chunk, MFMA_ITEM_QUERIES, true} : MfmaItemShape{chunk, MFMA_QBLOCK, false};
 }
 
 void launch_scan_mfma(const MfmaScanArgs& a, hipStream_t s) {
     if (a.nitems == 0 && !a.dev_nitems) return;
-    const unsigned nwg = (a.nitems + 3) / 4;
     static const unsigned per_cu_env = getenv("AUNCEL_AMD_MFMA_WG_PER_CU") ? (unsigned)atoi(getenv("AUNCEL_AMD_MFMA_WG_PER_CU")) : 0;
     const bool masked = a.thr != nullptr;
     const int ks = (int)mfma_ksteps(a.d);
     static const bool no_hint = getenv("AUNCEL_AMD_RESIDENT_GRIDS") != nullptr;
-    auto go = [&](auto kern) {
+    auto go = [&](auto kern, unsigned items_per_wg) {
         static const unsigned per_cu = blocks_per_cu(kern, 256);
-        const size_t hwg = ((size_t)a.hint_nitems + a.hint_nitems / 8 + 3) / 4;
+        const unsigned nwg = (a.nitems + items_per_wg - 1) / items_per_wg;
+        const size_t hwg = ((size_t)a.hint_nitems + a.hint_nitems / 8 + items_per_wg - 1) / items_per_wg;
         const unsigned hinted = (unsigned)((hwg + 7) / 8) * 8 + 8;
         const dim3 grid(a.dev_nitems ? (a.hint_nitems && !no_hint ? hinted : resident_grid(per_cu_env ? per_cu_env : per_cu))
                                      : a.xcd_chunks ? ((nwg + 7) / 8) * 8 : nwg),
                         block(256);
         LAUNCH(kern, grid, block, 0, s, a);
-#ifdef AUNCEL_AMD_SCAN_PROF
-        if (getenv("AUNCEL_AMD_SCAN_PROF")) {
-            unsigned long long c[8], z[8] = {0, 0, 0, 0, 0, 0, 0, 0};
-            (void)hipStreamSynchronize(s);
-            (void)hipMemcpyFromSymbol(c, HIP_SYMBOL(g_scan_prof), sizeof c);
-            (void)hipMemcpyToSymbol(HIP_SYMBOL(g_scan_prof), z, sizeof z);
-            if (c[0])
-                fprintf(stderr, "[scan prof] %s grid %u waves %llu items %llu | per wave (cycles of s_memtime): life %.0f first %.0f wait %.0f work %.0f "
-                        "item-prologue %.0f mask %.0f\n", masked ? "thr" : "dense", grid.x, c[0], c[7], (double)c[1] / c[0], (double)c[2] / c[0],
-                        (double)c[3] / c[0], (double)c[4] / c[0], (double)c[5] / c[0], (double)c[6] / c[0]);
-        }
-#endif
     };
     auto pick_ks = [&](auto metric, auto msk) {
         constexpr int M = decltype(metric)::value;
         constexpr bool K = decltype(msk)::value;
         switch (ks) {
-            case 1: return go(scan_mfma_kernel<M, K, 1>);
-            case 2: return go(scan_mfma_kernel<M, K, 2>);
-            case 3: return go(scan_mfma_kernel<M, K, 3>);
-            case 4: return go(scan_mfma_kernel<M, K, 4>);
-            default: return go(scan_mfma_kernel<M, K, 0>);
+            case 1: return go(scan_mfma_kernel<M, K, 1>, 4);
+            case 2: return go(scan_mfma_kernel<M, K, 2>, 4);
+            case 3: return go(scan_mfma_kernel<M, K, 3>, 4);
+            case 4: return go(scan_mfma_kernel<M, K, 4>, 4);
+            default: return go(scan_mfma_kernel<M, K, 0>, 4);
         }
     };
-    if (masked && mfma_thr_qblock(a.d, a.pipelined, a.exact_mask != 0) == 2 * MFMA_QBLOCK) {
-        if (a.metric == METRIC_L2) {
-            switch (ks) {
-                case 1: return go(scan_mfma_pair_kernel<METRIC_L2, 1>);
-                case 2: return go(scan_mfma_pair_kernel<METRIC_L2, 2>);
-                case 3: return go(scan_mfma_pair_kernel<METRIC_L2, 3>);
-                default: return go(scan_mfma_pair_kernel<METRIC_L2, 4>);
-            }
-        } else {
-            switch (ks) {
-                case 1: return go(scan_mfma_pair_kernel<METRIC_IP, 1>);
-                case 2: return go(scan_mfma_pair_kernel<METRIC_IP, 2>);
-                case 3: return go(scan_mfma_pair_kernel<METRIC_IP, 3>);
-                default: return go(scan_mfma_pair_kernel<METRIC_IP, 4>);
-            }
-        }
-    }
-    if ((a.pipelined & (masked ? 2 : 1)) && !(masked && a.exact_mask) && ks >= 1 && ks <= 4 && mfma_chunk() <= 512 && mfma_chunk_thr() <= 512) {
-        auto pick_thr = [&](auto metric, auto dense) {
+    if (mfma_item_shape(a.d, a.pipelined, masked, a.exact_mask != 0).shared) {
+        auto pick_shared = [&](auto metric, auto dense) {
             constexpr int M = decltype(metric)::value;
             constexpr bool D = decltype(dense)::value;
             switch (ks) {
-                case 1: return go(scan_mfma_thr_kernel<M, 1, D>);
-                case 2: return go(scan_mfma_thr_kernel<M, 2, D>);
-                case 3: return go(scan_mfma_thr_kernel<M, 3, D>);
-                default: return go(scan_mfma_thr_kernel<M, 4, D>);
+                case 1: return go(scan_mfma_shared_kernel<M, 1, D>, 1);
+                case 2: return go(scan_mfma_shared_kernel<M, 2, D>, 1);
+                case 3: return go(scan_mfma_shared_kernel<M, 3, D>, 1);
+                default: return go(scan_mfma_shared_kernel<M, 4, D>, 1);
             }
         };
         if (a.metric == METRIC_L2) {
-            if (masked) pick_thr(std::integral_constant<int, METRIC_L2>{}, std::false_type{});
-            else pick_thr(std::integral_constant<int, METRIC_L2>{}, std::true_type{});
+            if (masked) pick_shared(std::integral_constant<int, METRIC_L2>{}, std::false_type{});
+            else pick_shared(std::integral_constant<int, METRIC_L2>{}, std::true_type{});
         } else {
-            if (masked) pick_thr(std::integral_constant<int, METRIC_IP>{}, std::false_type{});
-            else pick_thr(std::integral_constant<int, METRIC_IP>{}, std::true_type{});
+            if (masked) pick_shared(std::integral_constant<int, METRIC_IP>{}, std::false_type{});
+            else pick_shared(std::integral_constant<int, METRIC_IP>{}, std::true_type{});
         }
         return;
     }
```

Result: slower. 2.074 million (-27.0%).
